# citibeth/spsparse

Hardware: NVIDIA B200
Metric: spgemm_intermediate_products_per_sec (higher is better)
Workload: dtype f64

## Files before the change

### spsparse_b200/csrc/radix_sort.cuh

```cuda
#pragma once
#include "common.cuh"

constexpr int RS_THREADS = 256;
#ifndef RS_IPT_N
#define RS_IPT_N 16
#endif
#ifndef RS_MIN_BLOCKS
#define RS_MIN_BLOCKS 3
#endif
constexpr int RS_IPT = RS_IPT_N;
constexpr int RS_HB = RS_IPT / 2;
constexpr int RS_TILE = RS_THREADS * RS_IPT;
constexpr int RS_WARPS = RS_THREADS / 32;
constexpr int RS_RADIX_BITS = 8;
constexpr int RS_RADIX = 1 << RS_RADIX_BITS;
constexpr int RS_NB = RS_RADIX + 1;
constexpr int RS_MAX_PASSES = 8;
#ifndef RS_LOOKBACK
#define RS_LOOKBACK 8
#endif
constexpr size_t RS_SMEM_BYTES =
    (size_t)RS_TILE * 16 + (size_t)RS_WARPS * RS_NB * sizeof(u32) + 64;

#define RS_WORD_AGG(c) ((c) + 1u)
// ... 218 lines not shown
                          input_kept(in, (u32)i, v[k]);
                key[h + k] = pack_key(hi[k], lo[k], in.bits_lo);
                valid_bits |= (ok ? 1u : 0u) << (h + k);
            }
        }
    } else if (BULK) {
        mbar_wait(&s_mbar[0], 0);
#pragma unroll
        for (int k = 0; k < RS_IPT; ++k) {
            const bool ok = wbase + (u64)k * 32 < n;
            key[k] = ok ? s_keys[warp * (32 * RS_IPT) + k * 32 + lane] : 0;
            valid_bits |= (ok ? 1u : 0u) << k;
        }
    } else {
#pragma unroll
        for (int k = 0; k < RS_IPT; ++k) {
            u64 i = wbase + (u64)k * 32;
            bool ok = i < n;
            key[k] = ok ? ld_stream_u64(a.keys_in + i) : 0;
            valid_bits |= (ok ? 1u : 0u) << k;
        }
#pragma unroll
        for (int k = 0; k < RS_IPT; ++k) {
            u64 i = wbase + (u64)k * 32;
            if (i < n && (lane & 15) == 0) asm volatile("prefetch.global.L2 [%0];" ::"l"(a.vals_in + i));
        }
    }

    u32 *mycnt = s_wcnt + warp * RS_NB;
    const u32 lt = lanemask_lt();
    unsigned short pos[RS_IPT];
#pragma unroll
    for (int k = 0; k < RS_IPT; ++k) {
        const bool ok = (valid_bits >> k) & 1u;
        const u32 d = (u32)((key[k] >> a.shift) & (RS_RADIX - 1));
        u32 peers;
        if (a.rank_mode == 0) {
            peers = __ballot_sync(SPB_FULL_MASK, ok);
#pragma unroll
            for (int b = 0; b < RS_RADIX_BITS; ++b) {
                int sgn;
                asm("bfe.s32 %0, %1, %2, 1;" : "=r"(sgn) : "r"(d), "r"(b));
                const u32 m = __ballot_sync(SPB_FULL_MASK, sgn != 0);
                peers &= ~(m ^ (u32)sgn);
            }
        } else {
            peers = __match_any_sync(SPB_FULL_MASK, ok ? d : (u32)RS_RADIX);
        }
        u32 leader = ok ? (u32)(__ffs(peers) - 1) : lane;
        u32 before = 0;
        if (ok && lane == leader) {
            before = mycnt[d];
            mycnt[d] = before + __popc(peers);
        }
        before = __shfl_sync(SPB_FULL_MASK, before, leader);
        pos[k] = (unsigned short)(before + __popc(peers & lt));
        __syncwarp();
    }
    __syncthreads();

    u32 total = 0;
#pragma unroll
    for (int w = 0; w < RS_WARPS; ++w) total += s_wcnt[w * RS_NB + tid];
    u32 *lb = a.lookback + (u64)tile * RS_RADIX + tid;
    st_relaxed_u32(lb, tile == 0 ? RS_WORD_INCL(total) : RS_WORD_AGG(total));
    u32 incl = warp_incl_scan(total);
    if (lane == 31) s_misc[1 + warp] = incl;
    __syncthreads();
    u32 lstart = incl - total;
    for (u32 w = 0; w < warp; ++w) lstart += s_misc[1 + w];
    const u32 nvalid_if_last = lstart + total;
    {
        u32 run = lstart;
#pragma unroll
        for (int w = 0; w < RS_WARPS; ++w) {
            u32 c = s_wcnt[w * RS_NB + tid];
            s_wcnt[w * RS_NB + tid] = run;
            run += c;
        }
    }
    if (tid == RS_RADIX - 1) s_misc[12] = nvalid_if_last;
    __syncthreads();
    const u32 nvalid = s_misc[12];

#pragma unroll
    for (int k = 0; k < RS_IPT; ++k) {
        if ((valid_bits >> k) & 1u) {
            u32 d = (u32)((key[k] >> a.shift) & (RS_RADIX - 1));
            u32 p = mycnt[d] + pos[k];
            pos[k] = (unsigned short)p;
            s_keys[p] = key[k];
        }
    }
    {
        const double *vsrc = PASS0 ? in.val : a.vals_in;
        double v[RS_IPT];
        if (BULK) {
            mbar_wait(&s_mbar[1], 0);
#pragma unroll
            for (int k = 0; k < RS_IPT; ++k) v[k] = s_vals[warp * (32 * RS_IPT) + k * 32 + lane];
            __syncthreads();
        } else {
#pragma unroll
            for (int k = 0; k < RS_IPT; ++k) {
                u64 i = wbase + (u64)k * 32;
                v[k] = ((valid_bits >> k) & 1u) ? ld_stream_f64(vsrc + i) : 0.0;
            }
        }
#pragma unroll
        for (int k = 0; k < RS_IPT; ++k)
            if ((valid_bits >> k) & 1u) s_vals[pos[k]] = v[k];
    }

    u32 excl = 0;
    if (tile > 0) {
        i64 p = (i64)tile - 1;
        bool done = false;
        while (!done) {
            u32 w[RS_LOOKBACK];
#pragma unroll
            for (int u = 0; u < RS_LOOKBACK; ++u)
                w[u] = (p - u >= 0) ? ld_relaxed_u32(a.lookback + (u64)(p - u) * RS_RADIX + tid) : RS_WORD_INCL(0u);
#pragma unroll
            for (int u = 0; u < RS_LOOKBACK; ++u) {
                if (done) break;
                while (!RS_READY(w[u])) w[u] = ld_relaxed_u32(a.lookback + (u64)(p - u) * RS_RADIX + tid);
                excl += RS_VALUE(w[u]);
                if (RS_IS_INCL(w[u])) done = true;
            }
            p -= RS_LOOKBACK;
        }
        st_relaxed_u32(lb, RS_WORD_INCL(excl + total));
    }
    const u32 gbase = a.bucket_start[tid] + excl - lstart;
    __syncthreads();
    s_wcnt[tid] = gbase;
    __syncthreads();

#pragma unroll
    for (int k = 0; k < RS_IPT; ++k) {
        u32 p = (u32)k * RS_THREADS + tid;
        if (p < nvalid) {
            u64 kk = s_keys[p];
            u32 dst = s_wcnt[(u32)((kk >> a.shift) & (RS_RADIX - 1))] + p;
            a.keys_out[dst] = kk;
            a.vals_out[dst] = s_vals[p];
        }
    }
}

constexpr int SG_THREADS = 256;
constexpr int SG_IPT = 8;
constexpr int SG_TILE = SG_THREADS * SG_IPT;
constexpr int SEG_MAX = 64;

constexpr int SG_CNT_SHIFT = 8;
__global__ void __launch_bounds__(SG_THREADS, 5) k_segment_sort(const u64 *__restrict__ keys_in, const double *__restrict__ vals_in,
                                                                const u32 *n_ptr, int bits_lo, u64 *keys_out, double *vals_out,
                                                                unsigned char *flags, u32 *long_count, u64 *tile_cnt = nullptr,
                                                                int keep_all = 0) {
    constexpr int W = SG_TILE + 2 * SEG_MAX;
    constexpr int ITS = (W + SG_THREADS - 1) / SG_THREADS;
    constexpr int NG = ITS * SG_THREADS / 32;
    __shared__ u64 s_key[W];
    __shared__ u32 s_col[W];
    __shared__ u32 s_hb[NG];
    __shared__ u32 s_last[NG];
    __shared__ u32 s_first[NG];
    const u32 n = *n_ptr;
    const u64 base = (u64)blockIdx.x * SG_TILE;
    if (base >= n) return;
    const u32 tid = threadIdx.x, lane = tid & 31, warp = tid >> 5;
    for (u32 q = tid; q < (u32)W; q += SG_THREADS) {
        const i64 g = (i64)base + (i64)q - SEG_MAX;
        s_key[q] = (g >= 0 && g < (i64)n) ? ld_stream_u64(keys_in + g) : ~0ull;
    }
#pragma unroll
    for (int k = 0; k < SG_IPT; ++k) {
        const u64 g = base + (u64)warp * 256 + (u64)k * 32 + lane;
        if (g < n && (lane & 15) == 0) asm volatile("prefetch.global.L2 [%0];" ::"l"(vals_in + g));
    }
    __syncthreads();
    const u64 lo_mask = (1ull << bits_lo) - 1;
#pragma unroll
    for (int it = 0; it < ITS; ++it) {
        const u32 q = (u32)it * SG_THREADS + tid;
        bool head = true;
        if (q < (u32)W) {
            const u64 kk = s_key[q];
            s_col[q] = (u32)(kk & lo_mask);
            head = q == 0 || (s_key[q - 1] >> bits_lo) != (kk >> bits_lo);
        }
        const u32 hb = __ballot_sync(SPB_FULL_MASK, head);
        if (lane == 0) {
            const u32 g = q >> 5;
            s_hb[g] = hb;
            s_last[g] = hb ? (g << 5) + 31 - __clz(hb) : 0;
            s_first[g] = hb ? (g << 5) + __ffs(hb) - 1 : 0xffffffffu;
        }
    }
    __syncthreads();
    if (warp == 0) {
        u32 carry = 0;
        for (int r = 0; r < (NG + 31) / 32; ++r) {
            const int g = r * 32 + (int)lane;
            const u32 mine = g < NG ? s_last[g] : 0;
            u32 inc = mine;
#pragma unroll
            for (int o = 1; o < 32; o <<= 1) {
                const u32 t = __shfl_up_sync(SPB_FULL_MASK, inc, o);
                if (lane >= (u32)o) inc = max(inc, t);
            }
            u32 exc = __shfl_up_sync(SPB_FULL_MASK, inc, 1);
            if (lane == 0) exc = 0;
            if (g < NG) s_last[g] = max(exc, carry);
            carry = max(carry, __shfl_sync(SPB_FULL_MASK, inc, 31));
        }
        carry = 0xffffffffu;
        for (int r = (NG + 31) / 32 - 1; r >= 0; --r) {
            const int g = r * 32 + (int)lane;
            const u32 mine = g < NG ? s_first[g] : 0xffffffffu;
            u32 inc = mine;
#pragma unroll
            for (int o = 1; o < 32; o <<= 1) {
                const u32 t = __shfl_down_sync(SPB_FULL_MASK, inc, o);
                if (lane + o < 32) inc = min(inc, t);
            }
            u32 exc = __shfl_down_sync(SPB_FULL_MASK, inc, 1);
            if (lane == 31) exc = 0xffffffffu;
            if (g < NG) s_first[g] = min(exc, carry);
            carry = min(carry, __shfl_sync(SPB_FULL_MASK, inc, 0));
        }
    }
    __syncthreads();
    u32 n_long = 0;
    i32 shift_by[SG_IPT];
    u32 cnt_at = 0, cnt_before = 0, cnt_after = 0;
    const u64 wbase = base + (u64)warp * 256;
#pragma unroll
    for (int k = 0; k < SG_IPT; ++k) {
        const u32 q = SEG_MAX + warp * 256 + (u32)k * 32 + lane;
        const u64 g = wbase + (u64)k * 32 + lane;
        shift_by[k] = 0;
        if (g < n) {
            bool head = true, rhead = false;
            const u32 grp = q >> 5, l = q & 31, hb = s_hb[grp];
            const u32 below = hb & (0xffffffffu >> (31 - l));
            const u32 st = below ? (grp << 5) + 31 - __clz(below) : s_last[grp];
            const u32 above = l < 31 ? hb & (0xffffffffu << (l + 1)) : 0u;
            const u32 nx = above ? (grp << 5) + __ffs(above) - 1 : s_first[grp];
            const bool is_long = nx - st > (u32)SEG_MAX;
            if (!is_long) {
                const u32 col = s_col[q];
                u32 before = 0, same = 0;
                for (u32 j = st; j < q; ++j) { before += s_col[j] <= col; same += s_col[j] == col; }
                for (u32 j = q + 1; j < nx; ++j) before += s_col[j] < col;
                shift_by[k] = (i32)(st + before) - (i32)q;
                head = keep_all || same == 0;
                rhead = before == 0;
            }
            if (flags) flags[g] = is_long;
            n_long += is_long;
            const u64 dst = (u64)((i64)g + shift_by[k]);
            const u32 inc = (head ? 1u : 0u) | (rhead ? 0x10000u : 0u);
            if (dst < wbase) cnt_before += inc;
            else if (dst >= wbase + 256) cnt_after += inc;
            else cnt_at += inc;
        }
    }
    if (tile_cnt) {
        const u32 a0 = __reduce_add_sync(SPB_FULL_MASK, cnt_at), a1 = __reduce_add_sync(SPB_FULL_MASK, cnt_before),
                  a2 = __reduce_add_sync(SPB_FULL_MASK, cnt_after);
        if (lane == 0) {
            u64 *t = tile_cnt + (wbase >> SG_CNT_SHIFT);
            if (a0) atomicAdd((ull *)t, (ull)(a0 & 0xffffu) | ((ull)(a0 >> 16) << 31));
            if (a1) atomicAdd((ull *)(t - 1), (ull)(a1 & 0xffffu) | ((ull)(a1 >> 16) << 31));
            if (a2) atomicAdd((ull *)(t + 1), (ull)(a2 & 0xffffu) | ((ull)(a2 >> 16) << 31));
        }
    }
    double v[SG_IPT];
#pragma unroll
    for (int k = 0; k < SG_IPT; ++k) {
        const u64 g = wbase + (u64)k * 32 + lane;
        v[k] = g < n ? ld_stream_f64(vals_in + g) : 0.0;
    }
#pragma unroll
    for (int k = 0; k < SG_IPT; ++k) {
        const u64 g = wbase + (u64)k * 32 + lane;
        if (g < n) {
            const u64 dst = (u64)((i64)g + shift_by[k]);
            keys_out[dst] = s_key[SEG_MAX + warp * 256 + k * 32 + lane];
            vals_out[dst] = v[k];
        }
    }
    n_long = __reduce_add_sync(SPB_FULL_MASK, n_long);
    if (n_long && lane == 0) atomicAdd(long_count, n_long);
}

static_assert(SG_TILE % 256 == 0 && (1 << SG_CNT_SHIFT) == 256, "a warp's 256 consecutive entries are one tile of the reduce pass");
#ifndef SGW_UNROLL_N
#define SGW_UNROLL_N 8
#endif
constexpr int SGW_UNROLL = SGW_UNROLL_N;
__global__ void __launch_bounds__(SG_THREADS, 6) k_segment_sort_walk(const u64 *__restrict__ keys_in, const double *__restrict__ vals_in,
                                                             const u32 *n_ptr, int bits_lo, u64 *keys_out, double *vals_out,
                                                             unsigned char *flags, u32 *long_count, u64 *tile_cnt = nullptr,
                                                             int keep_all = 0) {
    __shared__ u32 s_row[SG_TILE + 2 * SEG_MAX];
    __shared__ u32 s_col[SG_TILE + 2 * SEG_MAX];
    const u32 n = *n_ptr;
    const u64 base = (u64)blockIdx.x * SG_TILE;
    if (base >= n) return;
    const u32 tid = threadIdx.x;
    const u32 lo_mask = bits_lo >= 32 ? 0xffffffffu : (1u << bits_lo) - 1u;
    for (u32 q = tid; q < SG_TILE + 2 * SEG_MAX; q += SG_THREADS) {
        const i64 g = (i64)base + (i64)q - SEG_MAX;
        u32 row = 0xffffffffu, col = 0;
        if (g >= 0 && g < (i64)n) {
            const u64 key = ld_stream_u64(keys_in + g);
            row = (u32)(key >> bits_lo);
            col = (u32)key & lo_mask;
        }
        s_row[q] = row;
        s_col[q] = col;
    }
    const u32 lane = tid & 31, warp = tid >> 5;
    const u64 wbase = base + (u64)warp * 256;
    double v[SG_IPT];
#pragma unroll
    for (int k = 0; k < SG_IPT; ++k) {
        const u64 g = wbase + (u64)k * 32 + lane;
        v[k] = g < n ? ld_stream_f64(vals_in + g) : 0.0;
    }
    __syncthreads();
    u32 n_long = 0;
    u32 cnt_at = 0, cnt_before = 0, cnt_after = 0;
#pragma unroll
    for (int k = 0; k < SG_IPT; ++k) {
        const u32 q = SEG_MAX + warp * 256 + (u32)k * 32 + lane;
        const u64 g = wbase + (u64)k * 32 + lane;
        u64 dst = g;
        bool head = true, rhead = false;
        if (g < n) {
            const u32 row = s_row[q], col = s_col[q];
            u32 b = 0, f = 0, before = 0, same = 0;
            if (s_row[q - SEG_MAX] == row || s_row[q + SEG_MAX] == row) b = f = (u32)SEG_MAX;
            else {
#pragma unroll SGW_UNROLL
                for (b = 0; b < (u32)SEG_MAX; ++b) {
                    if (s_row[q - 1 - b] != row) break;
                    const u32 c = s_col[q - 1 - b];
                    before += c <= col;
                    same += c == col;
                }
#pragma unroll SGW_UNROLL
                for (f = 0; f < (u32)SEG_MAX; ++f) {
                    if (s_row[q + 1 + f] != row) break;
                    before += s_col[q + 1 + f] < col;
                }
            }
            const bool is_long = b == (u32)SEG_MAX || f == (u32)SEG_MAX || b + f + 1 > (u32)SEG_MAX;
            if (!is_long) {
                dst = g - b + before;
                head = keep_all || same == 0;
                rhead = before == 0;
            }
            keys_out[dst] = ((u64)row << bits_lo) | col;
            vals_out[dst] = v[k];
            if (flags) flags[g] = is_long;
            n_long += is_long;
            const u32 inc = (head ? 1u : 0u) | (rhead ? 0x10000u : 0u);
            if (dst < wbase) cnt_before += inc;
            else if (dst >= wbase + 256) cnt_after += inc;
            else cnt_at += inc;
        }
    }
    if (tile_cnt) {
        const u32 a0 = __reduce_add_sync(SPB_FULL_MASK, cnt_at), a1 = __reduce_add_sync(SPB_FULL_MASK, cnt_before),
                  a2 = __reduce_add_sync(SPB_FULL_MASK, cnt_after);
        if (lane == 0) {
            u64 *t = tile_cnt + (wbase >> SG_CNT_SHIFT);
            if (a0) atomicAdd((ull *)t, (ull)(a0 & 0xffffu) | ((ull)(a0 >> 16) << 31));
            if (a1) atomicAdd((ull *)(t - 1), (ull)(a1 & 0xffffu) | ((ull)(a1 >> 16) << 31));
            if (a2) atomicAdd((ull *)(t + 1), (ull)(a2 & 0xffffu) | ((ull)(a2 >> 16) << 31));
        }
    }
    n_long = __reduce_add_sync(SPB_FULL_MASK, n_long);
    if (n_long && lane == 0) atomicAdd(long_count, n_long);
}

constexpr int SGS_ROW = 5;
constexpr int SGS_H = SGS_ROW - 1;
constexpr int SGS_STEP = 32 - 2 * SGS_H;
constexpr int SGS_STEPS = (256 + SGS_STEP - 1) / SGS_STEP;
__global__ void __launch_bounds__(SG_THREADS, 6) k_segment_sort_shfl(const u64 *__restrict__ keys_in, const double *__restrict__ vals_in,
                                                                    const u32 *n_ptr, int bits_lo, u64 *keys_out, double *vals_out,
                                                                    unsigned char *flags, u32 *long_count, u64 *tile_cnt = nullptr,
                                                                    int keep_all = 0) {
    __shared__ u32 s_row[SG_TILE + 2 * SEG_MAX];
    __shared__ u32 s_col[SG_TILE + 2 * SEG_MAX];
    __shared__ double s_val[SG_TILE];
    const u32 n = *n_ptr;
    const u64 base = (u64)blockIdx.x * SG_TILE;
    if (base >= n) return;
    const u32 tid = threadIdx.x, lane = tid & 31, warp = tid >> 5;
    const u32 lo_mask = bits_lo >= 32 ? 0xffffffffu : (1u << bits_lo) - 1u;
    for (u32 q = tid; q < SG_TILE + 2 * SEG_MAX; q += SG_THREADS) {
        const i64 g = (i64)base + (i64)q - SEG_MAX;
        u32 row = 0xffffffffu, col = 0;
        if (g >= 0 && g < (i64)n) {
            const u64 key = ld_stream_u64(keys_in + g);
            row = (u32)(key >> bits_lo);
            col = (u32)key & lo_mask;
        }
        s_row[q] = row;
        s_col[q] = col;
    }
#pragma unroll
    for (int k = 0; k < SG_IPT; ++k) {
        const u32 e = (u32)k * SG_THREADS + tid;
        const u64 g = base + e;
        s_val[e] = g < n ? ld_stream_f64(vals_in + g) : 0.0;
    }
    __syncthreads();
    const u64 wbase = base + (u64)warp * 256;
    u32 n_long = 0;
    u32 cnt_at = 0, cnt_before = 0, cnt_after = 0;
    for (int t = 0; t < SGS_STEPS; ++t) {
        const i32 e = t * SGS_STEP + (i32)lane - SGS_H;
        const u32 q = (u32)(SEG_MAX + (i32)warp * 256 + e);
        const u64 g = wbase + (u64)(i64)e;
        const bool mine = lane >= (u32)SGS_H && lane < (u32)(32 - SGS_H) && e < 256 && g < n;
        const u32 row = s_row[q], col = s_col[q];
        const u32 hb = __ballot_sync(SPB_FULL_MASK, s_row[q - 1] != row);
        const u32 tail = __shfl_sync(SPB_FULL_MASK, (u32)(s_row[q + 1] != row), 31);
        const u64 z = ~((u64)hb | ((u64)tail << 32)) & 0x1ffffffffull;
        u64 run = z;
#pragma unroll
        for (int d = 1; d < SGS_ROW; ++d) run &= z >> d;
        u32 b = 0, f = 0, before = 0, same = 0;
        if (run == 0) {
#pragma unroll
            for (int d = 1; d < SGS_ROW; ++d) {
                const u32 ru = __shfl_up_sync(SPB_FULL_MASK, row, d), cu = __shfl_up_sync(SPB_FULL_MASK, col, d);
                const u32 rd = __shfl_down_sync(SPB_FULL_MASK, row, d), cd = __shfl_down_sync(SPB_FULL_MASK, col, d);
                const bool up = lane >= (u32)d && ru == row, dn = lane + d < 32u && rd == row;
                b += up;
                before += (up && cu <= col) + (dn && cd < col);
                same += up && cu == col;
                f += dn;
            }
        } else if (mine) {
            if (s_row[q - SEG_MAX] == row || s_row[q + SEG_MAX] == row) b = f = (u32)SEG_MAX;
            else {
                for (b = 0; b < (u32)SEG_MAX; ++b) {
                    if (s_row[q - 1 - b] != row) break;
                    const u32 c = s_col[q - 1 - b];
                    before += c <= col;
                    same += c == col;
                }
                for (f = 0; f < (u32)SEG_MAX; ++f) {
                    if (s_row[q + 1 + f] != row) break;
                    before += s_col[q + 1 + f] < col;
                }
            }
        }
        if (mine) {
            const bool is_long = b == (u32)SEG_MAX || f == (u32)SEG_MAX || b + f + 1 > (u32)SEG_MAX;
            u64 dst = g;
            bool head = true, rhead = false;
            if (!is_long) {
                dst = g - b + before;
                head = keep_all || same == 0;
                rhead = before == 0;
            }
            keys_out[dst] = ((u64)row << bits_lo) | col;
            vals_out[dst] = s_val[warp * 256 + (u32)e];
            if (flags) flags[g] = is_long;
            n_long += is_long;
            const u32 inc = (head ? 1u : 0u) | (rhead ? 0x10000u : 0u);
            if (dst < wbase) cnt_before += inc;
            else if (dst >= wbase + 256) cnt_after += inc;
            else cnt_at += inc;
        }
    }
    if (tile_cnt) {
        const u32 a0 = __reduce_add_sync(SPB_FULL_MASK, cnt_at), a1 = __reduce_add_sync(SPB_FULL_MASK, cnt_before),
                  a2 = __reduce_add_sync(SPB_FULL_MASK, cnt_after);
        if (lane == 0) {
            u64 *t = tile_cnt + (wbase >> SG_CNT_SHIFT);
            if (a0) atomicAdd((ull *)t, (ull)(a0 & 0xffffu) | ((ull)(a0 >> 16) << 31));
            if (a1) atomicAdd((ull *)(t - 1), (ull)(a1 & 0xffffu) | ((ull)(a1 >> 16) << 31));
            if (a2) atomicAdd((ull *)(t + 1), (ull)(a2 & 0xffffu) | ((ull)(a2 >> 16) << 31));
        }
    }
    n_long = __reduce_add_sync(SPB_FULL_MASK, n_long);
    if (n_long && lane == 0) atomicAdd(long_count, n_long);
}

__global__ void k_gather_flagged(const u64 *__restrict__ keys, const double *__restrict__ vals, const unsigned char *__restrict__ flags,
                                 const u64 *__restrict__ slot, u32 n, u64 *k_out, double *v_out) {
    for (u64 e = (u64)blockIdx.x * blockDim.x + threadIdx.x; e < n; e += (u64)gridDim.x * blockDim.x)
        if (flags[e]) { k_out[slot[e]] = keys[e]; v_out[slot[e]] = vals[e]; }
}
__global__ void k_scatter_flagged(const u64 *__restrict__ k_sorted, const double *__restrict__ v_sorted,
                                  const unsigned char *__restrict__ flags, const u64 *__restrict__ slot, u32 n, u64 *keys, double *vals) {
    for (u64 e = (u64)blockIdx.x * blockDim.x + threadIdx.x; e < n; e += (u64)gridDim.x * blockDim.x)
        if (flags[e]) { keys[e] = k_sorted[slot[e]]; vals[e] = v_sorted[slot[e]]; }
}
```

### spsparse_b200/csrc/reduce_segsort.cuh

```cuda
#pragma once
#include "radix_sort.cuh"
#include "reduce_by_key.cuh"

constexpr int RF_H = SEG_MAX;
constexpr int RF_W = RK_TILE + 2 * RF_H;
constexpr int RF_ITS = (RF_W + RK_THREADS - 1) / RK_THREADS;
constexpr int RF_SORTED = RK_TILE + RF_H + 1;
constexpr int RF_SLOTS = RF_SORTED + (RF_SORTED >> 3) + 1;

struct RfSmem {
    u64 raw[RF_W];
    u64 keys[RF_SLOTS];
    double vals[RF_SLOTS];
    u64 warp[RK_WARPS];
    u64 excl;
    u32 tile;
};

__global__ void __launch_bounds__(RK_THREADS, 4) k_reduce_segsort(ReduceArgs a, u32 *seg_long) {
    extern __shared__ __align__(16) unsigned char rf_smem[];
    RfSmem &s = *reinterpret_cast<RfSmem *>(rf_smem);
    const u32 tid = threadIdx.x, lane = tid & 31, warp = tid >> 5;
    const bool want_rows = a.row_start != nullptr;
    if (tid == 0) s.tile = atomicAdd(a.ticket, 1u);
    __syncthreads();
    const u32 tile = s.tile;
    const u32 n = *a.n_ptr;
    const u64 base = (u64)tile * RK_TILE;
    if (base >= n) return;
    const u32 tile_n = (n - base < (u64)RK_TILE) ? (u32)(n - base) : (u32)RK_TILE;

    double v[RF_ITS];
#pragma unroll
    for (int k = 0; k < RF_ITS; ++k) {
        const u32 q = (u32)k * RK_THREADS + tid;
        const i64 g = (i64)base + (i64)q - RF_H;
        const bool in = q < (u32)RF_W && g >= 0 && g < (i64)n;
        if (q < (u32)RF_W) s.raw[q] = in ? ld_stream_u64(a.keys + g) : ~0ull;
        v[k] = in ? ld_stream_f64(a.vals + g) : 0.0;
    }
    __syncthreads();

    const u64 lo_mask = (1ull << a.bits_lo) - 1;
    u32 n_long = 0;
#pragma unroll
    for (int k = 0; k < RF_ITS; ++k) {
        const u32 q = (u32)k * RK_THREADS + tid;
        if (q >= (u32)RF_W) continue;
        const u64 key = s.raw[q];
        if (key == ~0ull) continue;
        const u64 row = key >> a.bits_lo, col = key & lo_mask;
        u32 b = 0, f = 0, before = 0;
        bool cut = false;
        for (; b < (u32)SEG_MAX; ++b) {
            if (q < 1 + b) { cut = true; break; }
            const u64 kk = s.raw[q - 1 - b];
            if ((kk >> a.bits_lo) != row) break;
            before += (kk & lo_mask) <= col;
        }
        for (; f < (u32)SEG_MAX; ++f) {
            if (q + 1 + f >= (u32)RF_W) { cut = true; break; }
            const u64 kk = s.raw[q + 1 + f];
            if ((kk >> a.bits_lo) != row) break;
            before += (kk & lo_mask) < col;
        }
        const bool is_long = b == (u32)SEG_MAX || f == (u32)SEG_MAX || b + f + 1 > (u32)SEG_MAX;
        if (q >= (u32)RF_H && q < (u32)(RF_H + RK_TILE)) n_long += is_long;
        const u32 place = (cut || is_long) ? q : q - b + before;
        if (place + 1 >= (u32)RF_H && place + 1 < (u32)(RF_H + RF_SORTED)) {
            const u32 L = place + 1 - (u32)RF_H;
            s.keys[rk_phys(L)] = key;
            s.vals[rk_phys(L)] = v[k];
        }
    }
    n_long = __reduce_add_sync(SPB_FULL_MASK, n_long);
    if (n_long && lane == 0) atomicAdd(seg_long, n_long);
    __syncthreads();

    const u32 first = tid * RK_IPT;
    const u32 mine = first < tile_n ? (tile_n - first < (u32)RK_IPT ? tile_n - first : (u32)RK_IPT) : 0;
    u64 key[RK_IPT];
    double acc[RK_IPT];
    u32 head_bits = 0, rhead_bits = 0;
    if (mine) {
        const u64 prev = s.keys[rk_phys(first)];
#pragma unroll
        for (int j = 0; j < RK_IPT; ++j) {
            key[j] = s.keys[rk_phys(first + j + 1)];
            acc[j] = s.vals[rk_phys(first + j + 1)];
        }
        int cur = -1;
#pragma unroll
        for (int j = 0; j < RK_IPT; ++j) {
            if ((u32)j < mine) {
                const u64 before = j ? key[j - 1] : prev;
                const bool head = (a.policy == POLICY_KEEP_ALL) || (base + first + j == 0) || (key[j] != before);
                if (head) {
                    head_bits |= 1u << j;
                    if (want_rows && ((base + first + j == 0) || (key[j] >> a.bits_lo) != (before >> a.bits_lo)))
                        rhead_bits |= 1u << j;
                    cur = j;
                } else if (cur >= 0) {
                    const double vj = acc[j];
#pragma unroll
                    for (int h = 0; h < RK_IPT; ++h)
                        if (h == cur) {
                            if (a.policy == POLICY_ADD) acc[h] = __dadd_rn(acc[h], vj);
                            else if (a.policy == POLICY_REPLACE) acc[h] = vj;
                        }
                }
            }
        }
        if (cur >= 0 && mine == (u32)RK_IPT && (a.policy == POLICY_ADD || a.policy == POLICY_REPLACE)) {
            const u64 k0 = key[RK_IPT - 1];
            double sum = 0.0;
#pragma unroll
            for (int h = 0; h < RK_IPT; ++h) if (h == cur) sum = acc[h];
            u64 q = base + first + RK_IPT;
            while (q < n) {
                const u32 L = (u32)(q - base) + 1;
                if (L >= (u32)RF_SORTED) break;
                if (s.keys[rk_phys(L)] != k0) break;
                const double vq = s.vals[rk_phys(L)];
                if (a.policy == POLICY_ADD) sum = __dadd_rn(sum, vq); else sum = vq;
                ++q;
            }
#pragma unroll
            for (int h = 0; h < RK_IPT; ++h) if (h == cur) acc[h] = sum;
        }
    }
    const u32 emit_bits = head_bits;
    const u64 my = (u64)__popc(emit_bits) | ((u64)__popc(rhead_bits) << 32);
    const u64 incl = warp_incl_scan(my);
    if (lane == 31) s.warp[warp] = incl;
    __syncthreads();
    u64 wbefore = 0, total = 0;
#pragma unroll
    for (int w = 0; w < RK_WARPS; ++w) {
        const u64 t = s.warp[w];
        if ((u32)w < warp) wbefore += t;
        total += t;
    }
    const u64 before_me = wbefore + incl - my;
    const u32 tile_out = (u32)(total & 0xffffffffull);
    if (warp == 0) {
        const u64 packed = (total & 0xffffffffull) | ((total >> 32) << 31);
        const u64 excl0 = lookback_exclusive(a.state, tile, packed);
        if (lane == 0) {
            s.excl = excl0;
            if (base + RK_TILE >= n) {
                const u64 fin = excl0 + packed;
                const u32 n_out = (u32)(fin & 0x7fffffffull), n_rows = (u32)(fin >> 31);
                *a.out_count = n_out;
                if (want_rows) { *a.row_count = n_rows; a.row_start[n_rows] = n_out; }
            }
        }
    }
    {
        u32 slot = (u32)(before_me & 0xffffffffull);
#pragma unroll
        for (int j = 0; j < RK_IPT; ++j) {
            if ((emit_bits >> j) & 1u) {
                s.keys[slot] = key[j];
                s.vals[slot] = acc[j];
                ++slot;
            }
        }
    }
    __syncthreads();
    const u64 excl_rows = s.excl >> 31;
    const u64 excl = s.excl & 0x7fffffffull;
    if (rhead_bits) {
        u32 slot = (u32)(before_me & 0xffffffffull);
        u64 rslot = excl_rows + (before_me >> 32);
#pragma unroll
        for (int j = 0; j < RK_IPT; ++j) {
            if ((emit_bits >> j) & 1u) {
                if ((rhead_bits >> j) & 1u) {
                    a.row_start[rslot] = (u32)(excl + slot);
                    a.row_id[rslot] = (i32)(key[j] >> a.bits_lo);
                    ++rslot;
                }
                ++slot;
            }
        }
    }
    for (u32 t = tid; t < tile_out; t += RK_THREADS) {
        const u64 k = s.keys[t];
        a.out_hi[excl + t] = (i32)(k >> a.bits_lo);
        if (a.out_lo) a.out_lo[excl + t] = (i32)(k & lo_mask);
        a.out_val[excl + t] = s.vals[t];
    }
}
```

### spsparse_b200/csrc/spb_api.cu

```cuda
#include "../../include/spsparse_b200.h"

#include <cstdarg>
#include <cstdio>
#include <cstdlib>
#include <cstring>
#include <chrono>
#include <map>
#include <mutex>
#include <thread>
#include <unordered_map>
#include <vector>

#include "common.cuh"
#include "csr.cuh"
#include "gen.cuh"
#include "radix_sort.cuh"
#include "radix_sort9.cuh"
#include "reduce_by_key.cuh"
#include "reduce_segsort.cuh"
#include "reduce_warp.cuh"
#include "scan.cuh"
#include "spgemm.cuh"
#include "dense_ops.cuh"
#include "rowpart.cuh"

thread_local std::string g_last_error;

int spb_fail(int code, const char *fmt, ...) {
    char buf[1024];
    va_list ap;
    va_start(ap, fmt);
    vsnprintf(buf, sizeof buf, fmt, ap);
    va_end(ap);
    g_last_error = buf;
    return code;
}

static inline double now_ms() {
    return std::chrono::duration<double, std::milli>(std::chrono::steady_clock::now().time_since_epoch()).count();
}
static double g_alloc_ms = 0;
static int g_trace = -1;
static inline bool tracing() {
    if (g_trace < 0) g_trace = getenv("SPB_TRACE") ? 1 : 0;
    return g_trace == 1;
}

struct DevPool {
    std::multimap<size_t, void *> free_;
    std::unordered_map<void *, size_t> live_;
    std::mutex mu_;
    size_t cached_bytes = 0;

    static size_t round_up(size_t b) {
        if (b < 512) return 512;
        if (b < (1u << 20)) return (b + 511) & ~(size_t)511;
        return (b + (1u << 20) - 1) & ~(size_t)((1u << 20) - 1);
    }
    cudaError_t alloc(void **out, size_t bytes) {
        std::lock_guard<std::mutex> g(mu_);
        const size_t want = round_up(bytes);
        auto it = free_.lower_bound(want);
        if (it != free_.end() && it->first <= want + (want >= (64u << 20) ? want / 2 : want / 8)) {
            *out = it->second;
            live_[*out] = it->first;
            cached_bytes -= it->first;
            free_.erase(it);
            return cudaSuccess;
        }
        void *p = nullptr;
        cudaError_t e = cudaMalloc(&p, want);
        if (e != cudaSuccess) {
            cudaGetLastError();
            trim_locked();
            e = cudaMalloc(&p, want);
            if (e != cudaSuccess) return e;
        }
        live_[p] = want;
        *out = p;
        return cudaSuccess;
    }
    void release(void *p) {
        if (!p) return;
        std::lock_guard<std::mutex> g(mu_);
        auto it = live_.find(p);
        if (it == live_.end()) return;
        free_.insert({it->second, p});
        cached_bytes += it->second;
        live_.erase(it);
    }
    void trim_locked() {
        cudaDeviceSynchronize();
        for (auto &kv : free_) cudaFree(kv.second);
        free_.clear();
        cached_bytes = 0;
    }
    void destroy() {
        std::lock_guard<std::mutex> g(mu_);
        trim_locked();
        for (auto &kv : live_) cudaFree(kv.first);
        live_.clear();
    }
};

struct spb_ctx {
    int device;
    cudaStream_t stream;
    bool own_stream;
    int sm_count;
    u32 merge_max_products;
    u64 esc_chunk;
    u64 hash_min_products;
    int hash_variant;
    u64 launches;
    bool bulk_load;
    static constexpr int XFER_WORKERS = 8;
    int xfer_workers;
    static constexpr size_t XFER_CHUNK = 16u << 20;
    void *xfer_buf[XFER_WORKERS][2];
    cudaStream_t xfer_stream[XFER_WORKERS];
    cudaEvent_t xfer_ev[XFER_WORKERS][2];
    bool xfer_ready;
    DevPool pool;
};

struct spb_coo {
    int rank;
    u64 shape[2];
    u64 n;
    i32 *idx[2];
    double *val;
    int sort_order[2];
    bool owned;
    u32 *row_start;
    i32 *row_id;
    u32 nrows;
    bool rows_valid;
    u32 *dense_ptr;
    bool dense_ptr_owned;
    u32 *range_ptr;
    u64 range_lo, range_hi;
    u32 max_row_len;
};

struct Scratch {
    spb_ctx *ctx;
    std::vector<void *> ptrs;
    explicit Scratch(spb_ctx *c) : ctx(c) {}
    ~Scratch() { for (void *p : ptrs) ctx->pool.release(p); }
    template <typename T>
    int get(T **out, u64 count) {
        void *p = nullptr;
        size_t bytes = (size_t)(count ? count : 1) * sizeof(T);
        double t0 = tracing() ? now_ms() : 0;
        cudaError_t e = ctx->pool.alloc(&p, bytes);
        if (tracing()) { double dt = now_ms() - t0; g_alloc_ms += dt; if (dt > 1.0) fprintf(stderr, "[spb] pool.alloc(%zu MB) took %.2f ms\n", bytes >> 20, dt); }
        if (e != cudaSuccess) return spb_fail(SPB_ERR_CUDA, "device allocation of %zu bytes failed: %s", bytes, cudaGetErrorString(e));
        ptrs.push_back(p);
        *out = (T *)p;
        return 0;
    }
    template <typename T>
    int zeroed(T **out, u64 count) {
        CKR(get(out, count));
        CK(cudaMemsetAsync(*out, 0, (size_t)(count ? count : 1) * sizeof(T), ctx->stream));
        return 0;
    }
    void release(void *p) {
        for (size_t i = 0; i < ptrs.size(); ++i)
            if (ptrs[i] == p) { ctx->pool.release(p); ptrs.erase(ptrs.begin() + i); return; }
    }
    void keep(void *p) {
        for (size_t i = 0; i < ptrs.size(); ++i)
            if (ptrs[i] == p) { ptrs.erase(ptrs.begin() + i); return; }
    }
};

struct Timer {
    cudaStream_t s;
    std::vector<cudaEvent_t> ev;
    explicit Timer(cudaStream_t st) : s(st) {}
    ~Timer() { for (auto e : ev) cudaEventDestroy(e); }
    int mark() {
        cudaEvent_t e;
        cudaEventCreate(&e);
        cudaEventRecord(e, s);
        ev.push_back(e);
        return (int)ev.size() - 1;
    }
    float ms(int a, int b) {
        float t = 0;
        cudaEventSynchronize(ev[b]);
        cudaEventElapsedTime(&t, ev[a], ev[b]);
        return t;
    }
};

static inline u32 grid_for(u64 n, u32 threads, u32 cap) {
    u64 g = div_up(n ? n : 1, threads);
    return (u32)(g < cap ? g : cap);
}

static bool host_ptr_is_pinned(const void *p) {
    cudaPointerAttributes at;
    if (cudaPointerGetAttributes(&at, p) != cudaSuccess) { cudaGetLastError(); return false; }
    return at.type == cudaMemoryTypeHost || at.type == cudaMemoryTypeManaged;
}

static int xfer_setup(spb_ctx *c) {
    if (c->xfer_ready) return 0;
    {
        int want = getenv("SPB_XFER_WORKERS") ? atoi(getenv("SPB_XFER_WORKERS")) : (int)(std::thread::hardware_concurrency() / 2);
        c->xfer_workers = want < 1 ? 1 : (want > spb_ctx::XFER_WORKERS ? spb_ctx::XFER_WORKERS : want);
    }
    for (int w = 0; w < c->xfer_workers; ++w) {
        CK(cudaStreamCreateWithFlags(&c->xfer_stream[w], cudaStreamNonBlocking));
        for (int b = 0; b < 2; ++b) {
            CK(cudaHostAlloc(&c->xfer_buf[w][b], spb_ctx::XFER_CHUNK, cudaHostAllocDefault));
            CK(cudaEventCreateWithFlags(&c->xfer_ev[w][b], cudaEventDisableTiming));
        }
    }
    c->xfer_ready = true;
    return 0;
}

struct XferJob { void *dev; void *host; size_t bytes; };

static int staged_copy(spb_ctx *c, const XferJob *jobs, int njobs, bool to_device) {
    bool all_pinned = true;
    size_t total = 0;
    for (int j = 0; j < njobs; ++j) { if (jobs[j].bytes) { all_pinned = all_pinned && host_ptr_is_pinned(jobs[j].host); total += jobs[j].bytes; } }
    if (all_pinned || total < (4u << 20)) {
        for (int j = 0; j < njobs; ++j)
            if (jobs[j].bytes)
                CK(cudaMemcpyAsync(to_device ? jobs[j].dev : jobs[j].host, to_device ? jobs[j].host : jobs[j].dev, jobs[j].bytes,
                                   to_device ? cudaMemcpyHostToDevice : cudaMemcpyDeviceToHost, c->stream));
        CK(cudaStreamSynchronize(c->stream));
        return 0;
    }
    CKR(xfer_setup(c));
    struct Chunk { char *dev; char *host; size_t bytes; };
    std::vector<Chunk> chunks;
    for (int j = 0; j < njobs; ++j)
        for (size_t o = 0; o < jobs[j].bytes; o += spb_ctx::XFER_CHUNK)
            chunks.push_back({(char *)jobs[j].dev + o, (char *)jobs[j].host + o, std::min(spb_ctx::XFER_CHUNK, jobs[j].bytes - o)});
    const int NW = c->xfer_workers;
    cudaError_t err[spb_ctx::XFER_WORKERS];
    auto work = [&](int w) {
        cudaError_t e = cudaSetDevice(c->device);
        int b = 0;
        size_t pending_chunk[2] = {(size_t)-1, (size_t)-1};
        for (size_t k = w; k < chunks.size() && e == cudaSuccess; k += (size_t)NW, b ^= 1) {
            const Chunk &ch = chunks[k];
            if (to_device) {
                e = cudaEventSynchronize(c->xfer_ev[w][b]);
                if (e != cudaSuccess) break;
                memcpy(c->xfer_buf[w][b], ch.host, ch.bytes);
                e = cudaMemcpyAsync(ch.dev, c->xfer_buf[w][b], ch.bytes, cudaMemcpyHostToDevice, c->xfer_stream[w]);
                if (e == cudaSuccess) e = cudaEventRecord(c->xfer_ev[w][b], c->xfer_stream[w]);
            } else {
                e = cudaMemcpyAsync(c->xfer_buf[w][b], ch.dev, ch.bytes, cudaMemcpyDeviceToHost, c->xfer_stream[w]);
                if (e == cudaSuccess) e = cudaEventRecord(c->xfer_ev[w][b], c->xfer_stream[w]);
                pending_chunk[b] = k;
                const int o = b ^ 1;
                if (e == cudaSuccess && pending_chunk[o] != (size_t)-1) {
                    e = cudaEventSynchronize(c->xfer_ev[w][o]);
                    if (e == cudaSuccess) memcpy(chunks[pending_chunk[o]].host, c->xfer_buf[w][o], chunks[pending_chunk[o]].bytes);
                    pending_chunk[o] = (size_t)-1;
                }
            }
        }
        if (!to_device)
            for (int o = 0; o < 2 && e == cudaSuccess; ++o)
                if (pending_chunk[o] != (size_t)-1) {
                    e = cudaEventSynchronize(c->xfer_ev[w][o]);
                    if (e == cudaSuccess) memcpy(chunks[pending_chunk[o]].host, c->xfer_buf[w][o], chunks[pending_chunk[o]].bytes);
                }
        if (e == cudaSuccess) e = cudaStreamSynchronize(c->xfer_stream[w]);
        err[w] = e;
    };
    CK(cudaStreamSynchronize(c->stream));
    std::thread th[spb_ctx::XFER_WORKERS];
    for (int w = 1; w < NW; ++w) th[w] = std::thread(work, w);
    work(0);
    for (int w = 1; w < NW; ++w) th[w].join();
    for (int w = 0; w < NW; ++w)
        if (err[w] != cudaSuccess) return spb_fail(SPB_ERR_CUDA, "host transfer failed: %s", cudaGetErrorString(err[w]));
    return 0;
}

extern "C" {

const char *spb_last_error(void) { return g_last_error.c_str(); }
int spb_version(void) { return 100; }

int spb_ctx_create(int device, void *cuda_stream, spb_ctx **out) {
    if (!out) return spb_fail(SPB_ERR_ARG, "spb_ctx_create: out is null");
    int count = 0;
    cudaError_t e = cudaGetDeviceCount(&count);
    if (e != cudaSuccess || count == 0)
        return spb_fail(SPB_ERR_CUDA, "no CUDA device available (%s); spsparse_b200 has no CPU fallback",
                        cudaGetErrorString(e));
    if (device < 0 || device >= count) return spb_fail(SPB_ERR_ARG, "device %d out of range (%d devices)", device, count);
    CK(cudaSetDevice(device));
    struct Undo {
        spb_ctx *c;
        ~Undo() {
            if (!c) return;
            if (c->own_stream && c->stream) cudaStreamDestroy(c->stream);
            delete c;
        }
    } undo{new spb_ctx()};
    spb_ctx *c = undo.c;
    c->device = device;
    c->stream = nullptr;
    c->own_stream = (cuda_stream == nullptr);
    if (c->own_stream) CK(cudaStreamCreateWithFlags(&c->stream, cudaStreamNonBlocking));
    else c->stream = (cudaStream_t)cuda_stream;
    CK(cudaDeviceGetAttribute(&c->sm_count, cudaDevAttrMultiProcessorCount, device));
    CK(cudaFuncSetAttribute(k_radix_pass<true>, cudaFuncAttributeMaxDynamicSharedMemorySize, (int)RS_SMEM_BYTES));
    CK(cudaFuncSetAttribute(k_radix_pass<false>, cudaFuncAttributeMaxDynamicSharedMemorySize, (int)RS_SMEM_BYTES));
    CK(cudaFuncSetAttribute(k_reduce_segsort, cudaFuncAttributeMaxDynamicSharedMemorySize, (int)sizeof(RfSmem)));
    CK(cudaFuncSetAttribute(k_radix_pass9<true>, cudaFuncAttributeMaxDynamicSharedMemorySize, (int)R9_SMEM_BYTES));
    CK(cudaFuncSetAttribute(k_radix_pass9<false>, cudaFuncAttributeMaxDynamicSharedMemorySize, (int)R9_SMEM_BYTES));
    CK(cudaFuncSetAttribute(k_radix_pass<false, true>, cudaFuncAttributeMaxDynamicSharedMemorySize, (int)RS_SMEM_BYTES));
    CK(cudaFuncSetAttribute(k_radix_pass<true, true>, cudaFuncAttributeMaxDynamicSharedMemorySize, (int)RS_SMEM_BYTES));
    CK(cudaFuncSetAttribute(k_radix_pass9<true, true>, cudaFuncAttributeMaxDynamicSharedMemorySize, (int)R9_SMEM_BYTES));
    CK(cudaFuncSetAttribute(k_radix_pass9<false, true>, cudaFuncAttributeMaxDynamicSharedMemorySize, (int)R9_SMEM_BYTES));
    c->bulk_load = getenv("SPB_BULK_LOAD") ? atoi(getenv("SPB_BULK_LOAD")) != 0 : true;
    const char *s = getenv("SPB_MERGE_MAX_PRODUCTS");
    c->merge_max_products = s ? (u32)strtoul(s, nullptr, 10) : 1024u;
    s = getenv("SPB_ESC_CHUNK");
    c->esc_chunk = s ? strtoull(s, nullptr, 10) : (1ull << 27);
    c->launches = 0;
    c->xfer_ready = false;
    s = getenv("SPB_HASH_MIN_PRODUCTS");
    c->hash_min_products = s ? (strcmp(s, "off") == 0 ? ~0ull : strtoull(s, nullptr, 10)) : 512ull;
    s = getenv("SPB_HASH_VARIANT");
    c->hash_variant = s ? atoi(s) : 2;
    CK(cudaFuncSetAttribute(k_hash_symbolic, cudaFuncAttributeMaxDynamicSharedMemorySize, (int)(HASH_MAX_COLS / 8)));
    CK(cudaFuncSetAttribute(k_hash_numeric<1024, 10240, 16384>, cudaFuncAttributeMaxDynamicSharedMemorySize, (int)sizeof(HashSmem<1024, 10240, 16384>)));
    CK(cudaFuncSetAttribute(k_hash_numeric<512, 5120, 8192>, cudaFuncAttributeMaxDynamicSharedMemorySize, (int)sizeof(HashSmem<512, 5120, 8192>)));
    CK(cudaFuncSetAttribute(k_hash_numeric<256, 2560, 4096>, cudaFuncAttributeMaxDynamicSharedMemorySize, (int)sizeof(HashSmem<256, 2560, 4096>)));
    if (c->esc_chunk < 1) c->esc_chunk = 1;
    undo.c = nullptr;
    *out = c;
    return SPB_OK;
}

int spb_ctx_destroy(spb_ctx *ctx) {
    if (!ctx) return SPB_OK;
    cudaSetDevice(ctx->device);
    cudaStreamSynchronize(ctx->stream);
    if (ctx->xfer_ready)
        for (int w = 0; w < ctx->xfer_workers; ++w) {
            cudaStreamDestroy(ctx->xfer_stream[w]);
            for (int b = 0; b < 2; ++b) { cudaFreeHost(ctx->xfer_buf[w][b]); cudaEventDestroy(ctx->xfer_ev[w][b]); }
        }
    ctx->pool.destroy();
    if (ctx->own_stream) cudaStreamDestroy(ctx->stream);
    delete ctx;
    return SPB_OK;
}

int spb_ctx_sync(spb_ctx *ctx) {
    if (!ctx) return spb_fail(SPB_ERR_ARG, "null context");
    CK(cudaStreamSynchronize(ctx->stream));
    return SPB_OK;
}

int spb_ctx_trim(spb_ctx *ctx, uint64_t *released_bytes) {
    if (!ctx) return spb_fail(SPB_ERR_ARG, "null context");
    CK(cudaSetDevice(ctx->device));
    std::lock_guard<std::mutex> g(ctx->pool.mu_);
    if (released_bytes) *released_bytes = ctx->pool.cached_bytes;
    ctx->pool.trim_locked();
    return SPB_OK;
}

int spb_host_prefault(void *p, uint64_t bytes) {
    if (!p || !bytes) return SPB_OK;
    unsigned nt = std::thread::hardware_concurrency();
    if (nt > 16) nt = 16;
    if (bytes < (64ull << 20) || nt < 2) nt = 1;
    constexpr uint64_t PAGE = 4096;
    auto work = [=](unsigned t) {
        volatile char *c = static_cast<volatile char *>(p);
        const uint64_t a = bytes * t / nt, b = bytes * (t + 1) / nt;
        if (a < b) c[a] = 0;
        const uint64_t base = reinterpret_cast<uintptr_t>(p);
        for (uint64_t o = ((base + a + PAGE - 1) & ~(PAGE - 1)) - base; o < b; o += PAGE) c[o] = 0;
    };
    if (nt == 1) { work(0); return SPB_OK; }
    std::vector<std::thread> th;
    for (unsigned t = 1; t < nt; ++t) th.emplace_back(work, t);
    work(0);
    for (auto &x : th) x.join();
    return SPB_OK;
}

int spb_ctx_launch_count(const spb_ctx *ctx, uint64_t *launches) {
    if (!ctx || !launches) return spb_fail(SPB_ERR_ARG, "null argument");
    *launches = ctx->launches;
    return SPB_OK;
}

int spb_ctx_device(const spb_ctx *ctx, int *device, void **cuda_stream) {
    if (!ctx) return spb_fail(SPB_ERR_ARG, "null context");
    if (device) *device = ctx->device;
    if (cuda_stream) *cuda_stream = (void *)ctx->stream;
    return SPB_OK;
}

static int coo_new(spb_ctx *ctx, int rank, const u64 *shape, u64 n, bool allocate, spb_coo **out) {
    if (!ctx || !out || !shape) return spb_fail(SPB_ERR_ARG, "null argument");
    if (rank != 1 && rank != 2) return spb_fail(SPB_ERR_ARG, "rank must be 1 or 2 (got %d)", rank);
    for (int k = 0; k < rank; ++k)
        if (shape[k] > (1ull << 31)) return spb_fail(SPB_ERR_ARG, "extent %llu exceeds the int32 index range", (ull)shape[k]);
    if (n >= (1ull << 31)) return spb_fail(SPB_ERR_TOO_LARGE, "%llu entries: the reference's own cap is 2^31 (algorithm.hpp:419)", (ull)n);
    spb_coo *a = new spb_coo();
    a->rank = rank;
    a->shape[0] = shape[0];
    a->shape[1] = rank > 1 ? shape[1] : 1;
    a->n = n;
    a->idx[0] = a->idx[1] = nullptr;
    a->val = nullptr;
    a->sort_order[0] = -1;
    a->sort_order[1] = 0;
    a->owned = allocate;
    a->row_start = nullptr;
    a->row_id = nullptr;
    a->nrows = 0;
    a->rows_valid = false;
    a->dense_ptr = nullptr;
    a->dense_ptr_owned = true;
    a->range_ptr = nullptr;
    a->range_lo = a->range_hi = 0;
    a->max_row_len = 0;
    if (allocate) {
        size_t cnt = n ? n : 1;
        cudaError_t e = cudaSetDevice(ctx->device);
        for (int k = 0; k < rank && e == cudaSuccess; ++k) e = ctx->pool.alloc((void **)&a->idx[k], cnt * sizeof(i32));
        if (e == cudaSuccess) e = ctx->pool.alloc((void **)&a->val, cnt * sizeof(double));
        if (e != cudaSuccess) {
            for (int k = 0; k < 2; ++k) ctx->pool.release(a->idx[k]);
            ctx->pool.release(a->val);
            delete a;
            return spb_fail(SPB_ERR_CUDA, "device allocation for %llu entries failed: %s", (ull)n, cudaGetErrorString(e));
        }
    }
    *out = a;
    return SPB_OK;
}

static void drop_row_cache(spb_ctx *ctx, spb_coo *a) {
    if (ctx) {
        ctx->pool.release(a->row_start);
        ctx->pool.release(a->row_id);
        if (a->dense_ptr_owned) ctx->pool.release(a->dense_ptr);
        ctx->pool.release(a->range_ptr);
    }
    a->row_start = nullptr; a->row_id = nullptr; a->dense_ptr = nullptr; a->range_ptr = nullptr;
    a->rows_valid = false; a->nrows = 0; a->max_row_len = 0;
}

static void set_order(spb_coo *a, const int *so) {
    a->sort_order[0] = -1;
    a->sort_order[1] = 0;
    if (so && so[0] >= 0) {
        a->sort_order[0] = so[0];
        a->sort_order[1] = a->rank > 1 ? so[1] : 0;
    }
}

int spb_coo_alloc(spb_ctx *ctx, int rank, const uint64_t *shape, uint64_t n, spb_coo **out) {
    return coo_new(ctx, rank, shape, n, true, out);
}

int spb_coo_upload(spb_ctx *ctx, int rank, const uint64_t *shape, const int32_t *const *idx, const double *val,
                   uint64_t n, const int *sort_order, spb_coo **out) {
    if (n && (!idx || !val)) return spb_fail(SPB_ERR_ARG, "null data pointer");
    CKR(coo_new(ctx, rank, shape, n, true, out));
    spb_coo *a = *out;
    set_order(a, sort_order);
    XferJob jobs[3];
    int nj = 0;
    for (int k = 0; k < rank && n; ++k) {
        if (!idx[k]) { spb_coo_free(ctx, a); *out = nullptr; return spb_fail(SPB_ERR_ARG, "null index pointer for dimension %d", k); }
        jobs[nj++] = {a->idx[k], const_cast<int32_t *>(idx[k]), (size_t)n * sizeof(i32)};
    }
    if (n) jobs[nj++] = {a->val, const_cast<double *>(val), (size_t)n * sizeof(double)};
    const int rc = nj ? staged_copy(ctx, jobs, nj, true) : 0;
    if (rc) {
        spb_coo_free(ctx, a);
        *out = nullptr;
        return rc;
    }
    return SPB_OK;
}

int spb_coo_wrap_device(spb_ctx *ctx, int rank, const uint64_t *shape, int32_t *const *d_idx, double *d_val,
                        uint64_t n, const int *sort_order, spb_coo **out) {
    if (n && (!d_idx || !d_val)) return spb_fail(SPB_ERR_ARG, "null device pointer");
    CKR(coo_new(ctx, rank, shape, n, false, out));
    spb_coo *a = *out;
    for (int k = 0; k < rank; ++k) a->idx[k] = d_idx ? d_idx[k] : nullptr;
    a->val = d_val;
    set_order(a, sort_order);
    return SPB_OK;
}

int spb_coo_info(const spb_coo *a, int *rank, uint64_t *shape, uint64_t *n, int *sort_order) {
    if (!a) return spb_fail(SPB_ERR_ARG, "null array");
    if (rank) *rank = a->rank;
    for (int k = 0; k < a->rank; ++k) {
        if (shape) shape[k] = a->shape[k];
        if (sort_order) sort_order[k] = a->sort_order[k];
    }
    if (n) *n = a->n;
    return SPB_OK;
}

int spb_coo_device_ptrs(const spb_coo *a, int32_t **d_idx, double **d_val) {
    if (!a) return spb_fail(SPB_ERR_ARG, "null array");
    for (int k = 0; k < a->rank; ++k) if (d_idx) d_idx[k] = a->idx[k];
    if (d_val) *d_val = a->val;
    return SPB_OK;
}

int spb_coo_set_sorted(spb_coo *a, const int *sort_order) {
    if (!a) return spb_fail(SPB_ERR_ARG, "null array");
    if (a->rows_valid || a->dense_ptr)
        return spb_fail(SPB_ERR_ARG, "spb_coo_set_sorted: the array's row structure is already in use");
    set_order(a, sort_order);
    return SPB_OK;
}

int spb_coo_download(spb_ctx *ctx, const spb_coo *a, int32_t *const *idx, double *val) {
    if (!ctx || !a) return spb_fail(SPB_ERR_ARG, "null argument");
    CK(cudaSetDevice(ctx->device));
    XferJob jobs[3];
    int nj = 0;
    if (a->n) {
        for (int k = 0; k < a->rank; ++k)
            if (idx && idx[k]) jobs[nj++] = {a->idx[k], idx[k], (size_t)a->n * sizeof(i32)};
        if (val) jobs[nj++] = {a->val, val, (size_t)a->n * sizeof(double)};
    }
    if (nj) return staged_copy(ctx, jobs, nj, false);
    CK(cudaStreamSynchronize(ctx->stream));
    return SPB_OK;
}

int spb_coo_free(spb_ctx *ctx, spb_coo *a) {
    if (!a) return SPB_OK;
    if (a->owned && ctx) {
        for (int k = 0; k < 2; ++k) if (a->idx[k]) ctx->pool.release(a->idx[k]);
        if (a->val) ctx->pool.release(a->val);
    }
    drop_row_cache(ctx, a);
    delete a;
    return SPB_OK;
}

}

struct SortJob {
    SortInput in;
    int bits_hi;
    int policy;
};

template <typename InT, typename OutT>
static int exclusive_scan(spb_ctx *ctx, Scratch &ws, const InT *in, OutT *out, u64 n);

static int run_radix_passes(spb_ctx *ctx, Scratch &ws, int first_pass, int passes, u32 n_cap, const u32 *n_ptr,
                            u32 *hist, u64 *kA, double *vA, u64 *kB, double *vB, const SortInput *in0,
                            u64 **keys_sorted, double **vals_sorted, Timer *tm, int *mark_after_first, int shift0 = 0,
                            int digit_bits = RS_RADIX_BITS) {
    const u32 tiles = (u32)div_up(n_cap ? n_cap : 1, RS_TILE);
    const bool nine = digit_bits == R9_BITS;
    const u64 radix = nine ? R9_RADIX : RS_RADIX;
    u32 *lookback, *tickets;
    CKR(ws.zeroed(&lookback, (u64)passes * tiles * radix));
    CKR(ws.zeroed(&tickets, (u64)passes));
    u64 *kin = kA, *kout = kB;
    double *vin = vA, *vout = vB;
    for (int p = 0; p < passes; ++p) {
        PassArgs a;
        a.n_ptr = n_ptr;
        a.bucket_start = hist + (u64)p * radix;
        a.lookback = lookback + (u64)p * tiles * radix;
        a.ticket = tickets + p;
        a.shift = shift0 + p * digit_bits;
        a.rank_mode = getenv("SPB_RANK_MODE") ? atoi(getenv("SPB_RANK_MODE")) : 0;
        if (p == 0 && first_pass == 0) {
            a.keys_in = nullptr; a.vals_in = nullptr; a.keys_out = kA; a.vals_out = vA;
            const bool aligned = ((((uintptr_t)in0->hi) | ((uintptr_t)in0->lo) | ((uintptr_t)in0->val)) & 15u) == 0;
            const u32 tiles_bulk = (ctx->bulk_load && aligned) ? n_cap / RS_TILE : 0;
            if (tiles_bulk) {
                ++ctx->launches;
                if (nine) k_radix_pass9<true, true><<<tiles_bulk, RS_THREADS, R9_SMEM_BYTES, ctx->stream>>>(a, *in0);
                else k_radix_pass<true, true><<<tiles_bulk, RS_THREADS, RS_SMEM_BYTES, ctx->stream>>>(a, *in0);
            }
            if (tiles > tiles_bulk) {
                ++ctx->launches;
                if (nine) k_radix_pass9<true><<<tiles - tiles_bulk, RS_THREADS, R9_SMEM_BYTES, ctx->stream>>>(a, *in0);
                else k_radix_pass<true><<<tiles - tiles_bulk, RS_THREADS, RS_SMEM_BYTES, ctx->stream>>>(a, *in0);
            }
            kin = kA; vin = vA; kout = kB; vout = vB;
            if (tm) *mark_after_first = tm->mark();
        } else {
            a.keys_in = kin; a.vals_in = vin; a.keys_out = kout; a.vals_out = vout;
            SortInput dummy;
            memset(&dummy, 0, sizeof dummy);
            ++ctx->launches;
            if (ctx->bulk_load) {
                if (nine) k_radix_pass9<false, true><<<tiles, RS_THREADS, R9_SMEM_BYTES, ctx->stream>>>(a, dummy);
                else k_radix_pass<false, true><<<tiles, RS_THREADS, RS_SMEM_BYTES, ctx->stream>>>(a, dummy);
            } else {
                if (nine) k_radix_pass9<false><<<tiles, RS_THREADS, R9_SMEM_BYTES, ctx->stream>>>(a, dummy);
                else k_radix_pass<false><<<tiles, RS_THREADS, RS_SMEM_BYTES, ctx->stream>>>(a, dummy);
            }
            u64 *tk = kin; kin = kout; kout = tk;
            double *tv = vin; vin = vout; vout = tv;
        }
    }
    CK(cudaGetLastError());
    *keys_sorted = kin;
    *vals_sorted = vin;
    return 0;
}

static int sort_reduce(spb_ctx *ctx, const SortJob &job, i32 *out_hi, i32 *out_lo, double *out_val,
                       u32 *h_kept, u32 *h_out, spb_consolidate_stats *st, u32 *row_start = nullptr,
                       i32 *row_id = nullptr, u32 *h_rows = nullptr) {
    const SortInput &in = job.in;
    const u32 n = in.n;
    const int key_bits = job.bits_hi + in.bits_lo;
    int passes_full = (key_bits + RS_RADIX_BITS - 1) / RS_RADIX_BITS;
    if (passes_full < 1) passes_full = 1;
    if (passes_full > RS_MAX_PASSES) return spb_fail(SPB_ERR_ARG, "key of %d bits is too wide", key_bits);
    int passes_row = (job.bits_hi + RS_RADIX_BITS - 1) / RS_RADIX_BITS;
    if (passes_row < 1) passes_row = 1;
    const char *seg_env = getenv("SPB_SEGMENT_SORT");
    const bool seg_short = (double)n <= 16.0 * (double)in.extent_hi && n >= (1u << 23);
    const char *walk_env = getenv("SPB_SEGMENT_WALK");
    const bool seg_walk = walk_env ? atoi(walk_env) != 0 : (double)n <= 6.0 * (double)in.extent_hi;
    const bool seg_shfl = walk_env && atoi(walk_env) == 2;
    const bool seg = in.bits_lo > 0 && passes_full - passes_row >= 2 &&
                     (seg_env ? atoi(seg_env) != 0 : seg_short);
    const int cover_bits = seg ? job.bits_hi : key_bits;
    const char *r9_env = getenv("SPB_RADIX9");
    const int passes8 = seg ? passes_row : passes_full;
    const int passes9 = cover_bits > 0 ? (cover_bits + R9_BITS - 1) / R9_BITS : 1;
    const bool nine_wanted = r9_env ? atoi(r9_env) != 0 : (seg && !seg_env);
    const bool nine = nine_wanted && passes9 < passes8;
    const int digit_bits = nine ? R9_BITS : RS_RADIX_BITS;
    const int passes = nine ? passes9 : passes8;
    const int shift0 = seg ? in.bits_lo : 0;
    if (n >= (1u << 31)) return spb_fail(SPB_ERR_TOO_LARGE, "%u entries: one sort holds fewer than 2^31 (the reference's own cap, algorithm.hpp:419)", n);
    Scratch ws(ctx);
    Timer tm(ctx->stream);
    const int t0 = tm.mark();

    u32 *hist, *counters;
    u64 *first_kept;
    CKR(ws.zeroed(&hist, (u64)passes * (nine ? R9_RADIX : RS_RADIX)));
    CKR(ws.zeroed(&counters, 8));
    CKR(ws.get(&first_kept, 2));
    CK(cudaMemsetAsync(first_kept, 0xFF, 2 * sizeof(u64), ctx->stream));
    SortInput in0 = in;
    in0.first_kept = first_kept;
    const u32 sgrid = (u32)ctx->sm_count * 4;
    if (in.drop_nan) {
        ++ctx->launches, k_first_kept_key<<<grid_for(n, 256, sgrid * 2), 256, 0, ctx->stream>>>(in0, first_kept);
        ++ctx->launches, k_first_kept_pos<<<grid_for(n, 256, sgrid * 2), 256, 0, ctx->stream>>>(in0, first_kept);
    }
    const bool vec4 = ((((uintptr_t)in0.hi) | ((uintptr_t)in0.lo) | ((uintptr_t)in0.val)) & 15u) == 0 && n >= 4096 &&
                      !(getenv("SPB_VEC_LOAD") && atoi(getenv("SPB_VEC_LOAD")) == 0);
    if (nine) {
        ++ctx->launches;
        if (vec4) k_sort_hist_v4<9><<<grid_for(n / 4, 512, sgrid), 512, 0, ctx->stream>>>(in0, passes, shift0, hist, counters);
        else k_sort_hist9<<<grid_for(n, 512, sgrid), 512, 0, ctx->stream>>>(in0, passes, shift0, hist, counters);
        ++ctx->launches, k_bucket_starts9<<<passes, R9_RADIX / 2, 0, ctx->stream>>>(hist);
    } else {
        ++ctx->launches;
        if (vec4) k_sort_hist_v4<8><<<grid_for(n / 4, 512, sgrid), 512, 0, ctx->stream>>>(in0, passes, shift0, hist, counters);
        else k_sort_hist<<<grid_for(n, 512, sgrid), 512, 0, ctx->stream>>>(in0, passes, shift0, hist, counters);
        ++ctx->launches, k_bucket_starts<<<passes, RS_RADIX, 0, ctx->stream>>>(hist);
    }
    CK(cudaGetLastError());

    u64 *kA, *kB = nullptr, *ks;
    double *vA, *vB = nullptr, *vs;
    CKR(ws.get(&kA, n));
    CKR(ws.get(&vA, n));
    if (passes > 1 || seg) { CKR(ws.get(&kB, n)); CKR(ws.get(&vB, n)); }
    int t_p0 = t0;
    CKR(run_radix_passes(ctx, ws, 0, passes, n, counters, hist, kA, vA, kB, vB, &in0, &ks, &vs, &tm, &t_p0, shift0, digit_bits));
    const int t_passes = tm.mark();
    const char *fused_env = getenv("SPB_FUSED_REDUCE");
    bool fused = seg && seg_walk && fused_env && atoi(fused_env) != 0;
    u32 h[6];
    int t1 = t_passes, t2 = t_passes;
    u64 *const ks_rows = ks;
    double *const vs_rows = vs;
    bool long_rows_fixed = false;
    const int rw_mode = getenv("SPB_REDUCE_WARP") ? atoi(getenv("SPB_REDUCE_WARP")) : 1;
    const u32 wtiles = (u32)div_up(div_up(n ? n : 1, RW_TILE), RW_WARPS) * RW_WARPS;
    for (int attempt = 0;; ++attempt) {
        ks = ks_rows; vs = vs_rows;
        u64 *ko = (ks == kA) ? kB : kA;
        double *vo = (vs == vA) ? vB : vA;
        const u32 stiles = (u32)div_up(n, SG_TILE);
        u64 *tile_off = nullptr;
        if (seg && !fused) {
            if (!long_rows_fixed) {
                u64 *tile_cnt = nullptr;
                if (rw_mode == 1) {
                    CKR(ws.zeroed(&tile_cnt, (u64)wtiles + 2));
                    CKR(ws.get(&tile_off, (u64)wtiles + 2));
                }
                const int keep_all = job.policy == POLICY_KEEP_ALL;
                ++ctx->launches;
                if (seg_shfl) k_segment_sort_shfl<<<stiles, SG_THREADS, 0, ctx->stream>>>(ks, vs, counters, in.bits_lo, ko, vo, nullptr, counters + 5, tile_cnt, keep_all);
                else if (seg_walk) k_segment_sort_walk<<<stiles, SG_THREADS, 0, ctx->stream>>>(ks, vs, counters, in.bits_lo, ko, vo, nullptr, counters + 5, tile_cnt, keep_all);
                else k_segment_sort<<<stiles, SG_THREADS, 0, ctx->stream>>>(ks, vs, counters, in.bits_lo, ko, vo, nullptr, counters + 5, tile_cnt, keep_all);
                CK(cudaGetLastError());
                if (tile_cnt) CKR((exclusive_scan<u64, u64>(ctx, ws, tile_cnt, tile_off, (u64)wtiles + 1)));
            } else {
                const u32 n_kept = h[0], h_long = h[5];
                unsigned char *flags;
                u64 *slot, *lk, *lk2, *lks;
                double *lv, *lv2, *lvs;
                u32 *lhist, *lcount;
                CKR(ws.get(&flags, n_kept));
                CKR(ws.get(&slot, (u64)n_kept + 1));
                CK(cudaMemsetAsync(counters + 5, 0, sizeof(u32), ctx->stream));
                ++ctx->launches;
                if (seg_shfl) k_segment_sort_shfl<<<stiles, SG_THREADS, 0, ctx->stream>>>(ks, vs, counters, in.bits_lo, ko, vo, flags, counters + 5);
                else if (seg_walk) k_segment_sort_walk<<<stiles, SG_THREADS, 0, ctx->stream>>>(ks, vs, counters, in.bits_lo, ko, vo, flags, counters + 5);
                else k_segment_sort<<<stiles, SG_THREADS, 0, ctx->stream>>>(ks, vs, counters, in.bits_lo, ko, vo, flags, counters + 5);
                CKR((exclusive_scan<unsigned char, u64>(ctx, ws, flags, slot, n_kept)));
                CKR(ws.get(&lk, h_long)); CKR(ws.get(&lv, h_long)); CKR(ws.get(&lk2, h_long)); CKR(ws.get(&lv2, h_long));
                CKR(ws.zeroed(&lhist, (u64)passes_full * RS_RADIX));
                CKR(ws.zeroed(&lcount, 8));
                CK(cudaMemcpyAsync(lcount, &h_long, sizeof(u32), cudaMemcpyHostToDevice, ctx->stream));
                ++ctx->launches, k_gather_flagged<<<grid_for(n_kept, 256, sgrid * 4), 256, 0, ctx->stream>>>(ks, vs, flags, slot, n_kept, lk, lv);
                ++ctx->launches, k_keys_hist<<<grid_for(h_long, 512, sgrid), 512, 0, ctx->stream>>>(lk, h_long, passes_full, lhist);
                ++ctx->launches, k_bucket_starts<<<passes_full, RS_RADIX, 0, ctx->stream>>>(lhist);
                CKR(run_radix_passes(ctx, ws, 1, passes_full, h_long, lcount, lhist, lk, lv, lk2, lv2, nullptr, &lks, &lvs, nullptr, nullptr));
                ++ctx->launches, k_scatter_flagged<<<grid_for(n_kept, 256, sgrid * 4), 256, 0, ctx->stream>>>(lks, lvs, flags, slot, n_kept, ko, vo);
                CK(cudaGetLastError());
            }
            ks = ko; vs = vo;
        }
        t1 = tm.mark();

        const bool rwarp = !fused && (tile_off != nullptr || rw_mode == 2);
        const u32 rtiles = rwarp ? wtiles / RW_WARPS : (u32)div_up(n, RK_TILE);
        ReduceArgs ra;
        memset(&ra, 0, sizeof ra);
        ra.keys = ks; ra.vals = vs; ra.n_ptr = counters; ra.bits_lo = in.bits_lo; ra.policy = job.policy;
        ra.out_hi = out_hi; ra.out_lo = out_lo; ra.out_val = out_val; ra.out_count = counters + 2;
        if (tile_off) ra.state = tile_off;
        else CKR(ws.zeroed(&ra.state, rwarp ? (u64)wtiles : (u64)rtiles));
        CKR(ws.zeroed(&ra.ticket, 1));
        ra.long_cap = n / RK_LONG_RUN + 1;
        CKR(ws.get(&ra.long_list, 2ull * ra.long_cap));
        ra.long_count = counters + 3;
        ra.row_start = row_start; ra.row_id = row_id; ra.row_count = counters + 4;
        if (fused) {
            ++ctx->launches, k_reduce_segsort<<<rtiles, RK_THREADS, sizeof(RfSmem), ctx->stream>>>(ra, counters + 5);
        } else {
            if (rwarp && tile_off) ++ctx->launches, k_reduce_warp<false><<<rtiles, RW_THREADS, 0, ctx->stream>>>(ra);
            else if (rwarp) ++ctx->launches, k_reduce_warp<true><<<rtiles, RW_THREADS, 0, ctx->stream>>>(ra);
            else ++ctx->launches, k_reduce_by_key<MODE_CONSOLIDATE><<<rtiles, RK_THREADS, 0, ctx->stream>>>(ra);
            if (job.policy == POLICY_ADD || job.policy == POLICY_REPLACE)
                ++ctx->launches, k_long_runs<<<(u32)ctx->sm_count * 4, 256, 0, ctx->stream>>>(ra);
        }
        CK(cudaGetLastError());
        t2 = tm.mark();

        CK(cudaMemcpyAsync(h, counters, sizeof h, cudaMemcpyDeviceToHost, ctx->stream));
        CK(cudaStreamSynchronize(ctx->stream));
        if (h[5] && !h[1] && attempt == 0 && seg) {
            fused = false;
            long_rows_fixed = true;
            CK(cudaMemsetAsync(counters + 2, 0, 3 * sizeof(u32), ctx->stream));
            continue;
        }
        break;
    }
    if (h[1]) return spb_fail(SPB_ERR_ARG, "Sparse index out of bounds (an index is negative or >= its extent)");
    *h_kept = h[0];
    *h_out = h[2];
    if (h_rows) *h_rows = h[4];
    if (st) {
        st->n_in = n; st->n_kept = h[0]; st->n_out = h[2];
        st->key_bits = key_bits; st->passes = passes; st->digit_bits = digit_bits;
        st->ms_sort = tm.ms(t0, t1); st->ms_reduce = tm.ms(t1, t2); st->ms_total = tm.ms(t0, t2);
        st->ms_pass = passes > 1 ? tm.ms(t_p0, t_passes) / (float)(passes - 1) : 0.f;
    }
    return 0;
}

static int consolidate_core(spb_ctx *ctx, const spb_coo *in, const int *so, const int *ref_so, int policy,
                            bool drop_zero, int zero_nan, spb_coo **out, spb_consolidate_stats *st,
                            i32 *ext_lo = nullptr, double *ext_val = nullptr) {
    if (in->n >= (1ull << 31)) return spb_fail(SPB_ERR_TOO_LARGE, "%llu entries: one array holds fewer than 2^31 (the reference's own cap, algorithm.hpp:419)", (ull)in->n);
    spb_coo *r = nullptr;
    if (ext_lo && ext_val && in->rank == 2) {
        CKR(coo_new(ctx, in->rank, in->shape, in->n, false, &r));
        r->owned = true;
        if (ctx->pool.alloc((void **)&r->idx[so[0]], (in->n ? in->n : 1) * sizeof(i32)) != cudaSuccess) {
            delete r;
            return spb_fail(SPB_ERR_CUDA, "out of device memory");
        }
        r->idx[so[1]] = ext_lo;
        r->val = ext_val;
    } else {
        CKR(coo_new(ctx, in->rank, in->shape, in->n, true, &r));
    }
    set_order(r, so);
    if (st) memset(st, 0, sizeof *st);
    if (in->n == 0) { *out = r; return SPB_OK; }
    const int d0 = so[0], d1 = in->rank > 1 ? so[1] : -1;
    SortJob job;
    memset(&job, 0, sizeof job);
    job.in.hi = in->idx[d0];
    job.in.lo = d1 >= 0 ? in->idx[d1] : nullptr;
    job.in.val = in->val;
    job.in.n = (u32)in->n;
    job.in.bits_lo = d1 >= 0 ? bits_for(in->shape[d1]) : 0;
    job.in.extent_hi = (u32)(in->shape[d0] > 0xffffffffull ? 0xffffffffu : in->shape[d0]);
    job.in.extent_lo = d1 >= 0 ? (u32)in->shape[d1] : 1u;
    job.in.drop_zero = drop_zero ? 1 : 0;
    job.in.drop_nan = (drop_zero && zero_nan) ? 1 : 0;
    const int r0 = ref_so[0], r1 = in->rank > 1 ? ref_so[1] : -1;
    job.in.ref_hi = in->idx[r0];
    job.in.ref_lo = r1 >= 0 ? in->idx[r1] : nullptr;
    job.in.ref_bits_lo = r1 >= 0 ? bits_for(in->shape[r1]) : 0;
    job.bits_hi = bits_for(in->shape[d0]);
    job.policy = policy;
    u32 kept = 0, nout = 0, nrows = 0;
    if (in->rank == 2) {
        const u64 cap = (in->n < in->shape[d0] ? in->n : in->shape[d0]) + 1;
        if (ctx->pool.alloc((void **)&r->row_start, cap * sizeof(u32)) != cudaSuccess ||
            ctx->pool.alloc((void **)&r->row_id, cap * sizeof(i32)) != cudaSuccess) {
            spb_coo_free(ctx, r);
            return spb_fail(SPB_ERR_CUDA, "out of device memory");
        }
    }
    int rc = sort_reduce(ctx, job, r->idx[d0], d1 >= 0 ? r->idx[d1] : nullptr, r->val, &kept, &nout, st,
                         r->row_start, r->row_id, &nrows);
    if (rc) { spb_coo_free(ctx, r); return rc; }
    r->n = nout;
    if (in->rank == 2) {
        r->nrows = nrows;
        r->rows_valid = true;
        if (nout == 0) { const u32 z = 0; cudaMemcpyAsync(r->row_start, &z, sizeof z, cudaMemcpyHostToDevice, ctx->stream); }
    }
    *out = r;
    return SPB_OK;
}

static int check_order(const spb_coo *a, const int *so, const char *what) {
    if (!so) return spb_fail(SPB_ERR_ARG, "%s: sort_order is null", what);
    for (int k = 0; k < a->rank; ++k)
        if (a->n && !a->idx[k]) return spb_fail(SPB_ERR_ARG, "%s: array is in compressed (pointer) form", what);
    bool seen[2] = {false, false};
    for (int k = 0; k < a->rank; ++k) {
        if (so[k] < 0 || so[k] >= a->rank || seen[so[k]])
            return spb_fail(SPB_ERR_ARG, "%s: sort_order is not a permutation of the dimensions", what);
        seen[so[k]] = true;
    }
    return 0;
}

struct RowIndex {
    u32 *start;
    i32 *id;
    u32 nrows;
};

static int build_row_index(spb_ctx *ctx, const spb_coo *a_const, RowIndex *ri) {
    spb_coo *a = const_cast<spb_coo *>(a_const);
    if (!a->rows_valid && a->n && !a->idx[a->sort_order[0]])
        return spb_fail(SPB_ERR_ARG, "array in compressed (pointer) form has no row list; use it as the B operand only");
    if (!a->rows_valid) {
        const u32 n = (u32)a->n;
        const i32 *hi = a->idx[a->sort_order[0]];
        Scratch ws(ctx);
        u32 *rs = nullptr;
        i32 *rid = nullptr;
        CK(ctx->pool.alloc((void **)&rs, ((u64)n + 1) * sizeof(u32)));
        if (ctx->pool.alloc((void **)&rid, ((u64)n + 1) * sizeof(i32)) != cudaSuccess) {
            ctx->pool.release(rs);
            return spb_fail(SPB_ERR_CUDA, "out of device memory (row list of %u entries)", n);
        }
        a->row_start = rs; a->row_id = rid;
        u32 *count, *ticket;
        u64 *state;
        const u32 tiles = (u32)div_up(n ? n : 1, RH_TILE);
        CKR(ws.zeroed(&count, 1));
        CKR(ws.zeroed(&ticket, 1));
        CKR(ws.zeroed(&state, tiles));
        if (n) ++ctx->launches, k_row_heads<<<tiles, RH_THREADS, 0, ctx->stream>>>(hi, n, a->row_start, a->row_id, count, state, ticket);
        ++ctx->launches, k_row_sentinel<<<1, 1, 0, ctx->stream>>>(a->row_start, count, n);
        CK(cudaGetLastError());
        CK(cudaMemcpyAsync(&a->nrows, count, sizeof(u32), cudaMemcpyDeviceToHost, ctx->stream));
        CK(cudaStreamSynchronize(ctx->stream));
        a->rows_valid = true;
    }
    ri->start = a->row_start;
    ri->id = a->row_id;
    ri->nrows = a->nrows;
    return 0;
}

template <typename InT, typename OutT>
static int exclusive_scan(spb_ctx *ctx, Scratch &ws, const InT *in, OutT *out, u64 n) {
    if (n == 0) { CK(cudaMemsetAsync(out, 0, sizeof(OutT), ctx->stream)); return 0; }
    const u32 tiles = (u32)div_up(n, SC_TILE);
    u64 *state;
    u32 *ticket;
    CKR(ws.zeroed(&state, tiles));
    CKR(ws.zeroed(&ticket, 1));
    ++ctx->launches, k_exclusive_scan<InT, OutT><<<tiles, SC_THREADS, 0, ctx->stream>>>(in, out, n, state, ticket);
    CK(cudaGetLastError());
    return 0;
}

static int build_dense_ptr(spb_ctx *ctx, const spb_coo *a_const, u64 extent, u32 **ptr_out) {
    spb_coo *a = const_cast<spb_coo *>(a_const);
    if (!a->dense_ptr) {
        RowIndex ri;
        CKR(build_row_index(ctx, a, &ri));
        CK(ctx->pool.alloc((void **)&a->dense_ptr, (extent + 2) * sizeof(u32)));
        Scratch ws(ctx);
        DpGap *gaps = nullptr;
        u32 *n_gaps = nullptr;
        if (ri.nrows && extent + 1 - ri.nrows >= DP_LONG_GAP) {
            CKR(ws.get(&gaps, (extent + 1) / DP_LONG_GAP + 1));
            CKR(ws.zeroed(&n_gaps, 1));
        }
        ++ctx->launches;
        if (ri.nrows) k_dense_ptr_from_rows<<<grid_for(ri.nrows, 256, (u32)ctx->sm_count * 16), 256, 0, ctx->stream>>>(ri.start, ri.id, ri.nrows, (u32)a->n, extent, a->dense_ptr, gaps, n_gaps);
        else k_fill_u32<<<grid_for(extent + 1, 256, (u32)ctx->sm_count * 16), 256, 0, ctx->stream>>>(a->dense_ptr, extent + 1, 0u);
        if (gaps) ++ctx->launches, k_fill_gaps<<<(u32)ctx->sm_count * 8, 256, 0, ctx->stream>>>(gaps, n_gaps, a->dense_ptr);
        CK(cudaGetLastError());
    }
    *ptr_out = a->dense_ptr;
    return 0;
}

static int densify(spb_ctx *ctx, Scratch &ws, const spb_coo *v, u64 dim, double **dense, unsigned char **mask, u32 *bad) {
    CKR(ws.zeroed(dense, dim));
    if (mask) CKR(ws.zeroed(mask, dim));
    if (v->n) ++ctx->launches, k_densify<<<grid_for(v->n, 256, 1u << 16), 256, 0, ctx->stream>>>(v->idx[0], v->val, v->n, dim, *dense, mask ? *mask : nullptr, bad);
    CK(cudaGetLastError());
    return 0;
}
static int bad_scale_vector() {
    return spb_fail(SPB_ERR_ARG, "a scale vector (or a vector operand flagged sorted) is not strictly ascending in its index: the "
                    "reference joins these as sorted lists without repeats (xiter.hpp:146, 201)");
}

static int esc_sort_reduce(spb_ctx *ctx, u64 *kA, double *vA, u32 count, int key_bits, int kbits,
                           const MMOperands &m, u32 row_lo, i32 *t_row, i32 *t_k, double *t_v, u32 *h_out) {
    Scratch ws(ctx);
    int passes = (key_bits + RS_RADIX_BITS - 1) / RS_RADIX_BITS;
    if (passes < 1) passes = 1;
    u32 *hist, *counters;
    CKR(ws.zeroed(&hist, (u64)passes * RS_RADIX));
    CKR(ws.zeroed(&counters, 8));
    CK(cudaMemcpyAsync(counters, &count, sizeof(u32), cudaMemcpyHostToDevice, ctx->stream));
    ++ctx->launches, k_keys_hist<<<grid_for(count, 512, (u32)ctx->sm_count * 4), 512, 0, ctx->stream>>>(kA, count, passes, hist);
    ++ctx->launches, k_bucket_starts<<<passes, RS_RADIX, 0, ctx->stream>>>(hist);
    u64 *kB, *ks;
    double *vB, *vs;
    CKR(ws.get(&kB, count));
    CKR(ws.get(&vB, count));
    {
        const u32 tiles = (u32)div_up(count, RS_TILE);
        u32 *lookback, *tickets;
        CKR(ws.zeroed(&lookback, (u64)passes * tiles * RS_RADIX));
        CKR(ws.zeroed(&tickets, (u64)passes));
        u64 *kin = kA, *kout = kB;
        double *vin = vA, *vout = vB;
        SortInput dummy;
        memset(&dummy, 0, sizeof dummy);
        for (int p = 0; p < passes; ++p) {
            PassArgs a;
            a.keys_in = kin; a.vals_in = vin; a.keys_out = kout; a.vals_out = vout;
            a.n_ptr = counters;
            a.bucket_start = hist + (u64)p * RS_RADIX;
            a.lookback = lookback + (u64)p * tiles * RS_RADIX;
            a.ticket = tickets + p;
            a.shift = p * RS_RADIX_BITS;
            a.rank_mode = 0;
        a.rank_mode = getenv("SPB_RANK_MODE") ? atoi(getenv("SPB_RANK_MODE")) : 0;
            ++ctx->launches;
            if (ctx->bulk_load) k_radix_pass<false, true><<<tiles, RS_THREADS, RS_SMEM_BYTES, ctx->stream>>>(a, dummy);
            else k_radix_pass<false><<<tiles, RS_THREADS, RS_SMEM_BYTES, ctx->stream>>>(a, dummy);
            u64 *tk = kin; kin = kout; kout = tk;
            double *tv = vin; vin = vout; vout = tv;
        }
        ks = kin; vs = vin;
        CK(cudaGetLastError());
    }
    const u32 rtiles = (u32)div_up(count, RK_TILE);
    ReduceArgs ra;
    memset(&ra, 0, sizeof ra);
    ra.keys = ks; ra.vals = vs; ra.n_ptr = counters; ra.bits_lo = kbits; ra.policy = POLICY_ADD;
    ra.out_hi = t_row; ra.out_lo = t_k; ra.out_val = t_v; ra.out_count = counters + 2;
    CKR(ws.zeroed(&ra.state, rtiles));
    CKR(ws.zeroed(&ra.ticket, 1));
    ra.row_ids = m.arow_id; ra.row_base = (i32)row_lo; ra.si = m.si; ra.sk = m.sk; ra.C = m.C;
    ++ctx->launches, k_reduce_by_key<MODE_ESC><<<rtiles, RK_THREADS, 0, ctx->stream>>>(ra);
    CK(cudaGetLastError());
    CK(cudaMemcpyAsync(h_out, counters + 2, sizeof(u32), cudaMemcpyDeviceToHost, ctx->stream));
    CK(cudaStreamSynchronize(ctx->stream));
    return 0;
}

struct EscChunk { i32 *row; i32 *k; double *v; u32 n; };

static size_t ballast_for_blocks(int blocks_per_sm, size_t static_smem) {
    if (blocks_per_sm <= 0) return 0;
    const size_t per = (size_t)(227 * 1024) / (size_t)blocks_per_sm;
    return per > static_smem + 1024 ? per - static_smem - 1024 : 0;
}
template <typename K> static int allow_ballast(K kernel) {
    static thread_local const void *done[16];
    static thread_local int n = 0;
    for (int i = 0; i < n; ++i) if (done[i] == (const void *)kernel) return 0;
    CK(cudaFuncSetAttribute(kernel, cudaFuncAttributeMaxDynamicSharedMemorySize, 200 * 1024));
    if (n < 16) done[n++] = (const void *)kernel;
    return 0;
}

struct PreScale {
    const double *sj;
    const unsigned char *sj_mask;
};

static int multiply_core(spb_ctx *ctx, double C, const spb_coo *si, const spb_coo *A, int a_row_dim,
                         const spb_coo *sj, const spb_coo *B, int b_inner_dim, const spb_coo *sk,
                         spb_coo *out, spb_mm_stats *st, Timer &tm, int t_begin, bool symbolic_only = false,
                         const PreScale *pre = nullptr) {
    Scratch ws(ctx);
    const int a_in = 1 - a_row_dim, b_col = 1 - b_inner_dim;
    const u64 m_rows = A->shape[a_row_dim], n_inner = A->shape[a_in], n_cols = B->shape[b_col];
    MMOperands m;
    memset(&m, 0, sizeof m);
    m.C = C;
    m.debug = getenv("SPB_MERGE_DEBUG") ? atoi(getenv("SPB_MERGE_DEBUG")) : 0;
    m.a_j = A->idx[a_in]; m.a_val = A->val; m.nnz_a = (u32)A->n;
    RowIndex ri;
    CKR(build_row_index(ctx, A, &ri));
    m.arow_id = ri.id; m.arow_start = ri.start; m.nrows = ri.nrows;
    u32 *bptr;
    CKR(build_dense_ptr(ctx, B, n_inner, &bptr));
    m.bptr = bptr; m.b_k = B->idx[b_col]; m.b_val = B->val;
    double *d;
    unsigned char *mask;
    u32 *bad_vec;
    CKR(ws.zeroed(&bad_vec, 1));
    if (si) { CKR(densify(ctx, ws, si, m_rows, &d, nullptr, bad_vec)); m.si = d; }
    if (pre) { m.sj = pre->sj; m.sj_mask = pre->sj_mask; }
    else if (sj) { CKR(densify(ctx, ws, sj, n_inner, &d, &mask, bad_vec)); m.sj = d; m.sj_mask = mask; }
    if (sk) { CKR(densify(ctx, ws, sk, n_cols, &d, nullptr, bad_vec)); m.sk = d; }
    const int t_prep = tm.mark();
    double h0 = now_ms();
    if (tracing()) fprintf(stderr, "[spb] mm: prepare done (host), alloc so far %.2f ms\n", g_alloc_ms);

    const u32 nrows = m.nrows;
    u32 *row_cnt;
    u64 *ent_off = nullptr, *esc_f = nullptr, *esc_off, *c_ptr;
    unsigned char *row_cls;
    ull *stats;
    CKR(ws.get(&row_cls, nrows));
    CKR(ws.zeroed(&row_cnt, (u64)nrows + 1));
    ull *mstats;
    CKR(ws.zeroed(&stats, 8));
    CKR(ws.zeroed(&mstats, (u64)MC_STRIPES * 8));
    const u32 cap = (u32)ctx->sm_count * 32;
    {
        const double avg_a_len = nrows ? (double)m.nnz_a / (double)nrows : 0.0;
// ... 1391 lines not shown
```

Baseline: 43.64 billion.

## Replace last radix pass with in-block group sort over low row bits

Adds a k_group_sort kernel that, when groups of consecutive row-bit buckets are expected to fit in a 4096-entry shared-memory tile, sorts each group in shared memory on up to 9 low row bits and then runs the per-row column walk. This lets the global radix sort skip one full pass over the keys and values. It also removes the unused fused reduce kernel and the shuffle segment-sort variant, and moves the row walk into a shared helper. Groups that overflow the tile or contain long rows fall back to the existing long-row path, which adds complexity and can cost extra work on skewed inputs.

Measured after the change: 37.92 billion (median of 6 runs). 13.1% lower.

```diff
diff --git a/spsparse_b200/csrc/group_sort.cuh b/spsparse_b200/csrc/group_sort.cuh
--- /dev/null
+++ b/spsparse_b200/csrc/group_sort.cuh
@@ -0,0 +1,271 @@
+#pragma once
+#include "radix_sort.cuh"
+
+constexpr int GS_THREADS = 256;
+constexpr int GS_WARPS = GS_THREADS / 32;
+constexpr int GS_CAP = 4096;
+constexpr int GS_IPT = GS_CAP / GS_THREADS;
+constexpr int GS_TILE = GS_CAP;
+constexpr int GS_MAX_BITS = 9;
+constexpr int GS_RADIX = 1 << GS_MAX_BITS;
+constexpr int GS_TC = (GS_TILE + GS_CAP) / 256 + 1;
+static_assert(GS_TILE >= GS_CAP && (1 << SG_CNT_SHIFT) == 256, "see the carry-in rule in k_group_sort");
+constexpr u32 GS_RES_DST = 0x1fffu, GS_RES_HEAD = 0x4000u, GS_RES_RHEAD = 0x8000u;
+static_assert(GS_CAP <= (int)GS_RES_DST + 1, "a destination inside the group fits GS_RES_DST");
+#ifndef GS_MIN_BLOCKS
+#define GS_MIN_BLOCKS 2
+#endif
+
+struct GsSmem {
+    u32 row[GS_CAP + 2 * SEG_MAX];
+    u32 col[GS_CAP + 2 * SEG_MAX];
+    double val[GS_CAP];
+    unsigned short res[GS_CAP];
+    u32 cnt[GS_WARPS * GS_RADIX / 2];
+    u32 hb[GS_TILE / 32];
+    u64 tc[GS_TC];
+    u32 misc[16];
+};
+
+__device__ __forceinline__ u32 gs_next_head(const u32 *hb, u32 from, u32 len) {
+    const u32 lane = threadIdx.x & 31, nw = (len + 31) >> 5;
+    for (u32 w0 = from >> 5; w0 < nw; w0 += 32) {
+        const u32 w = w0 + lane;
+        u32 bits = w < nw ? hb[w] : 0u;
+        if (w == (from >> 5)) bits &= 0xffffffffu << (from & 31);
+        const u32 any = __ballot_sync(SPB_FULL_MASK, bits != 0);
+        if (any) {
+            const u32 l = __ffs(any) - 1;
+            return ((w0 + l) << 5) + __ffs(__shfl_sync(SPB_FULL_MASK, bits, l)) - 1;
+        }
+    }
+    return len;
+}
+
+__device__ void gs_leave(const u64 *__restrict__ keys_in, const double *__restrict__ vals_in, u64 lo, u64 hi, u64 gkey,
+                         bool starts_group, int keep_all, u64 base, u64 *keys_out, double *vals_out, unsigned char *flags,
+                         u32 *long_count, u64 *tc) {
+    const u32 tid = threadIdx.x;
+    for (u64 j = lo + tid; j < hi; j += GS_THREADS) {
+        if (flags) { keys_out[j] = keys_in[j]; vals_out[j] = vals_in[j]; flags[j] = 1; }
+        else { keys_out[j] = gkey; vals_out[j] = 0.0; }
+    }
+    if (tid == 0) atomicAdd(long_count, (u32)(hi - lo));
+    const u64 t0 = lo >> SG_CNT_SHIFT, t1 = (hi - 1) >> SG_CNT_SHIFT;
+    for (u64 t = t0 + tid; t <= t1; t += GS_THREADS) {
+        u64 c = 0;
+        if (keep_all) c = min(hi, (t + 1) << SG_CNT_SHIFT) - max(lo, t << SG_CNT_SHIFT);
+        else if (starts_group && t == t0) c = 1;
+        if (starts_group && t == t0) c |= 1ull << 31;
+        if (c) atomicAdd((ull *)&tc[t - (base >> SG_CNT_SHIFT)], (ull)c);
+    }
+}
+
+__global__ void __launch_bounds__(GS_THREADS, GS_MIN_BLOCKS) k_group_sort(const u64 *__restrict__ keys_in, const double *__restrict__ vals_in,
+                                                                         const u32 *n_ptr, int bits_lo, int gbits, u64 *keys_out, double *vals_out,
+                                                                         unsigned char *flags, u32 *long_count, u64 *tile_cnt, int keep_all) {
+    extern __shared__ __align__(16) unsigned char gs_raw[];
+    GsSmem &S = *reinterpret_cast<GsSmem *>(gs_raw);
+    const u32 n = *n_ptr;
+    const u64 base = (u64)blockIdx.x * GS_TILE;
+    if (base >= n) return;
+    const u32 tid = threadIdx.x, lane = tid & 31, warp = tid >> 5;
+    const u32 tlen = n - base < (u64)GS_TILE ? (u32)(n - base) : (u32)GS_TILE;
+    const int gshift = bits_lo + gbits;
+    const u32 lo_mask = bits_lo >= 32 ? 0xffffffffu : (1u << bits_lo) - 1u;
+    const u32 gmask = (1u << gbits) - 1u;
+
+    u32 *s_grp = S.row;
+    if (tid == 0) s_grp[0] = base ? (u32)(keys_in[base - 1] >> gshift) : 0xffffffffu;
+    for (int t = tid; t < GS_TC; t += GS_THREADS) S.tc[t] = 0;
+#pragma unroll
+    for (int k = 0; k < GS_IPT; ++k) {
+        const u32 i = (u32)k * GS_THREADS + tid;
+        if (i < tlen) s_grp[1 + i] = (u32)(ld_stream_u64(keys_in + base + i) >> gshift);
+    }
+    __syncthreads();
+#pragma unroll
+    for (int k = 0; k < GS_IPT; ++k) {
+        const u32 i = (u32)k * GS_THREADS + tid;
+        const u32 hb = __ballot_sync(SPB_FULL_MASK, i < tlen && s_grp[1 + i] != s_grp[i]);
+        if (lane == 0) S.hb[i >> 5] = hb;
+    }
+    __syncthreads();
+    u32 cs = gs_next_head(S.hb, 0, tlen);
+    if (cs > 0) {
+        const u32 grp = s_grp[1];
+        bool over = cs == tlen && base + tlen < n;
+        if (!over) {
+            const u64 ge = base + cs;
+            over = ge > (u64)GS_CAP && (u32)(keys_in[ge - GS_CAP - 1] >> gshift) == grp;
+        }
+        if (over) gs_leave(keys_in, vals_in, base, base + cs, (u64)grp << gshift, false, keep_all, base, keys_out, vals_out, flags, long_count, S.tc);
+    }
+
+    while (cs < tlen) {
+        const u64 gs = base + cs;
+        const u32 grp = (u32)(keys_in[gs] >> gshift);
+        const u64 gkey = (u64)grp << gshift;
+        const u32 nx = gs_next_head(S.hb, cs + 1, tlen);
+        u64 ge = base + nx;
+        if (nx == tlen && base + tlen < n) {
+            const u64 hs = base + tlen, lim = min((u64)n, gs + GS_CAP + 1);
+            u32 first = (u32)(lim - hs);
+#pragma unroll
+            for (int k = 0; k < GS_IPT; ++k) {
+                const u64 j = hs + (u64)k * GS_THREADS + tid;
+                if (j < lim && (u32)(ld_stream_u64(keys_in + j) >> gshift) != grp) first = min(first, (u32)(j - hs));
+            }
+            first = __reduce_min_sync(SPB_FULL_MASK, first);
+            if (lane == 0) S.misc[8 + warp] = first;
+            __syncthreads();
+            first = S.misc[8];
+#pragma unroll
+            for (int w = 1; w < GS_WARPS; ++w) first = min(first, S.misc[8 + w]);
+            ge = hs + first;
+        }
+        if (ge - gs > (u64)GS_CAP) {
+            gs_leave(keys_in, vals_in, gs, base + tlen, gkey, true, keep_all, base, keys_out, vals_out, flags, long_count, S.tc);
+            break;
+        }
+        const u32 m = (u32)(ge - gs);
+        const u32 K = (m + GS_THREADS - 1) / GS_THREADS;
+        __syncthreads();
+
+        u32 dig[GS_IPT], col[GS_IPT];
+        u32 valid_bits = 0;
+#pragma unroll
+        for (int k = 0; k < GS_IPT; ++k) {
+            const u32 i = warp * 32 * K + (u32)k * 32 + lane;
+            const bool ok = (u32)k < K && i < m;
+            const u64 key = ok ? ld_stream_u64(keys_in + gs + i) : 0;
+            dig[k] = (u32)(key >> bits_lo) & gmask;
+            col[k] = (u32)key & lo_mask;
+            valid_bits |= (ok ? 1u : 0u) << k;
+            if (ok && (lane & 15) == 0) asm volatile("prefetch.global.L2 [%0];" ::"l"(vals_in + gs + i));
+        }
+        for (int t = tid; t < GS_WARPS * GS_RADIX / 2; t += GS_THREADS) S.cnt[t] = 0;
+        if (tid < (u32)SEG_MAX) { S.row[tid] = 0xffffffffu; S.row[SEG_MAX + m + tid] = 0xffffffffu; }
+        __syncthreads();
+
+        unsigned short *mycnt = reinterpret_cast<unsigned short *>(S.cnt) + warp * GS_RADIX;
+        const u32 lt = lanemask_lt();
+        unsigned short pos[GS_IPT];
+#pragma unroll
+        for (int k = 0; k < GS_IPT; ++k) {
+            pos[k] = 0;
+            if (__any_sync(SPB_FULL_MASK, (valid_bits >> k) & 1u)) {
+                const bool ok = (valid_bits >> k) & 1u;
+                u32 peers = __ballot_sync(SPB_FULL_MASK, ok);
+#pragma unroll
+                for (int b = 0; b < GS_MAX_BITS; ++b) {
+                    int sgn;
+                    asm("bfe.s32 %0, %1, %2, 1;" : "=r"(sgn) : "r"(dig[k]), "r"(b));
+                    const u32 mb = __ballot_sync(SPB_FULL_MASK, sgn != 0);
+                    peers &= ~(mb ^ (u32)sgn);
+                }
+                const u32 leader = ok ? (u32)(__ffs(peers) - 1) : lane;
+                u32 before = 0;
+                if (ok && lane == leader) {
+                    before = mycnt[dig[k]];
+                    mycnt[dig[k]] = (unsigned short)(before + __popc(peers));
+                }
+                before = __shfl_sync(SPB_FULL_MASK, before, leader);
+                pos[k] = (unsigned short)(before + __popc(peers & lt));
+                __syncwarp();
+            }
+        }
+        __syncthreads();
+
+        {
+            u32 tot0 = 0, tot1 = 0;
+#pragma unroll
+            for (int w = 0; w < GS_WARPS; ++w) {
+                const u32 c = S.cnt[w * (GS_RADIX / 2) + tid];
+                tot0 += c & 0xffffu;
+                tot1 += c >> 16;
+            }
+            const u32 pair = tot0 + tot1, incl = warp_incl_scan(pair);
+            if (lane == 31) S.misc[warp] = incl;
+            __syncthreads();
+            u32 run0 = incl - pair;
+            for (u32 w = 0; w < warp; ++w) run0 += S.misc[w];
+            u32 run1 = run0 + tot0;
+#pragma unroll
+            for (int w = 0; w < GS_WARPS; ++w) {
+                const u32 c = S.cnt[w * (GS_RADIX / 2) + tid];
+                S.cnt[w * (GS_RADIX / 2) + tid] = (run0 & 0xffffu) | (run1 << 16);
+                run0 += c & 0xffffu;
+                run1 += c >> 16;
+            }
+        }
+        __syncthreads();
+
+        {
+#pragma unroll
+            for (int k = 0; k < GS_IPT; ++k) {
+                if ((valid_bits >> k) & 1u) {
+                    const u32 p = (u32)mycnt[dig[k]] + pos[k];
+                    pos[k] = (unsigned short)p;
+                    S.row[SEG_MAX + p] = dig[k];
+                    S.col[SEG_MAX + p] = col[k];
+                }
+            }
+            double v[GS_IPT];
+#pragma unroll
+            for (int k = 0; k < GS_IPT; ++k) {
+                const u32 i = warp * 32 * K + (u32)k * 32 + lane;
+                v[k] = ((valid_bits >> k) & 1u) ? ld_stream_f64(vals_in + gs + i) : 0.0;
+            }
+#pragma unroll
+            for (int k = 0; k < GS_IPT; ++k)
+                if ((valid_bits >> k) & 1u) S.val[pos[k]] = v[k];
+        }
+        __syncthreads();
+
+        bool any_long = false;
+#pragma unroll 1
+        for (u32 p = tid; p < m; p += GS_THREADS) {
+            u32 b, f, before, same;
+            const bool is_long = sg_row_walk(S.row, S.col, SEG_MAX + p, b, f, before, same);
+            any_long |= is_long;
+            S.res[p] = (unsigned short)(((p - b + before) & GS_RES_DST) |
+                                        (keep_all || same == 0 ? GS_RES_HEAD : 0u) |
+                                        (before == 0 ? GS_RES_RHEAD : 0u));
+        }
+        const bool left = __syncthreads_or(any_long);
+        if (left) gs_leave(keys_in, vals_in, gs, ge, gkey, true, keep_all, base, keys_out, vals_out, flags, long_count, S.tc);
+#pragma unroll
+        for (int k = 0; k < GS_IPT; ++k) {
+            const u32 p0 = (u32)k * GS_THREADS + warp * 32, p = p0 + lane;
+            if (!__any_sync(SPB_FULL_MASK, !left && p < m)) continue;
+            u32 cnt_at = 0, cnt_before = 0, cnt_after = 0;
+            if (p < m) {
+                const u32 r = S.res[p];
+                const u64 d = gs + (r & GS_RES_DST);
+                keys_out[d] = gkey | ((u64)S.row[SEG_MAX + p] << bits_lo) | S.col[SEG_MAX + p];
+                vals_out[d] = S.val[p];
+                if (flags) flags[gs + p] = 0;
+                const u32 inc = ((r & GS_RES_HEAD) ? 1u : 0u) | ((r & GS_RES_RHEAD) ? 0x10000u : 0u);
+                const u64 t = d >> SG_CNT_SHIFT, tw = (gs + p0) >> SG_CNT_SHIFT;
+                if (t < tw) cnt_before = inc;
+                else if (t > tw) cnt_after = inc;
+                else cnt_at = inc;
+            }
+            const u32 a0 = __reduce_add_sync(SPB_FULL_MASK, cnt_at), a1 = __reduce_add_sync(SPB_FULL_MASK, cnt_before),
+                      a2 = __reduce_add_sync(SPB_FULL_MASK, cnt_after);
+            if (lane == 0) {
+                u64 *t = S.tc + (((gs + p0) >> SG_CNT_SHIFT) - (base >> SG_CNT_SHIFT));
+                if (a0) atomicAdd((ull *)t, (ull)(a0 & 0xffffu) | ((ull)(a0 >> 16) << 31));
+                if (a1) atomicAdd((ull *)(t - 1), (ull)(a1 & 0xffffu) | ((ull)(a1 >> 16) << 31));
+                if (a2) atomicAdd((ull *)(t + 1), (ull)(a2 & 0xffffu) | ((ull)(a2 >> 16) << 31));
+            }
+        }
+        cs = nx;
+    }
+    if (tile_cnt) {
+        __syncthreads();
+        for (int t = tid; t < GS_TC; t += GS_THREADS)
+            if (S.tc[t]) atomicAdd((ull *)(tile_cnt + (base >> SG_CNT_SHIFT) + t), (ull)S.tc[t]);
+    }
+}
diff --git a/spsparse_b200/csrc/radix_sort.cuh b/spsparse_b200/csrc/radix_sort.cuh
--- a/spsparse_b200/csrc/radix_sort.cuh
+++ b/spsparse_b200/csrc/radix_sort.cuh
@@ -544,6 +544,27 @@
 #define SGW_UNROLL_N 8
 #endif
 constexpr int SGW_UNROLL = SGW_UNROLL_N;
+
+__device__ __forceinline__ bool sg_row_walk(const u32 *s_row, const u32 *s_col, u32 q, u32 &b, u32 &f, u32 &before, u32 &same) {
+    const u32 row = s_row[q], col = s_col[q];
+    before = same = 0;
+    if (s_row[q - SEG_MAX] == row || s_row[q + SEG_MAX] == row) b = f = (u32)SEG_MAX;
+    else {
+#pragma unroll SGW_UNROLL
+        for (b = 0; b < (u32)SEG_MAX; ++b) {
+            if (s_row[q - 1 - b] != row) break;
+            const u32 c = s_col[q - 1 - b];
+            before += c <= col;
+            same += c == col;
+        }
+#pragma unroll SGW_UNROLL
+        for (f = 0; f < (u32)SEG_MAX; ++f) {
+            if (s_row[q + 1 + f] != row) break;
+            before += s_col[q + 1 + f] < col;
+        }
+    }
+    return b == (u32)SEG_MAX || f == (u32)SEG_MAX || b + f + 1 > (u32)SEG_MAX;
+}
 __global__ void __launch_bounds__(SG_THREADS, 6) k_segment_sort_walk(const u64 *__restrict__ keys_in, const double *__restrict__ vals_in,
                                                              const u32 *n_ptr, int bits_lo, u64 *keys_out, double *vals_out,
                                                              unsigned char *flags, u32 *long_count, u64 *tile_cnt = nullptr,
@@ -585,23 +606,8 @@
         bool head = true, rhead = false;
         if (g < n) {
             const u32 row = s_row[q], col = s_col[q];
-            u32 b = 0, f = 0, before = 0, same = 0;
-            if (s_row[q - SEG_MAX] == row || s_row[q + SEG_MAX] == row) b = f = (u32)SEG_MAX;
-            else {
-#pragma unroll SGW_UNROLL
-                for (b = 0; b < (u32)SEG_MAX; ++b) {
-                    if (s_row[q - 1 - b] != row) break;
-                    const u32 c = s_col[q - 1 - b];
-                    before += c <= col;
-                    same += c == col;
-                }
-#pragma unroll SGW_UNROLL
-                for (f = 0; f < (u32)SEG_MAX; ++f) {
-                    if (s_row[q + 1 + f] != row) break;
-                    before += s_col[q + 1 + f] < col;
-                }
-            }
-            const bool is_long = b == (u32)SEG_MAX || f == (u32)SEG_MAX || b + f + 1 > (u32)SEG_MAX;
+            u32 b, f, before, same;
+            const bool is_long = sg_row_walk(s_row, s_col, q, b, f, before, same);
             if (!is_long) {
                 dst = g - b + before;
                 head = keep_all || same == 0;
@@ -631,115 +637,6 @@
     if (n_long && lane == 0) atomicAdd(long_count, n_long);
 }
 
-constexpr int SGS_ROW = 5;
-constexpr int SGS_H = SGS_ROW - 1;
-constexpr int SGS_STEP = 32 - 2 * SGS_H;
-constexpr int SGS_STEPS = (256 + SGS_STEP - 1) / SGS_STEP;
-__global__ void __launch_bounds__(SG_THREADS, 6) k_segment_sort_shfl(const u64 *__restrict__ keys_in, const double *__restrict__ vals_in,
-                                                                    const u32 *n_ptr, int bits_lo, u64 *keys_out, double *vals_out,
-                                                                    unsigned char *flags, u32 *long_count, u64 *tile_cnt = nullptr,
-                                                                    int keep_all = 0) {
-    __shared__ u32 s_row[SG_TILE + 2 * SEG_MAX];
-    __shared__ u32 s_col[SG_TILE + 2 * SEG_MAX];
-    __shared__ double s_val[SG_TILE];
-    const u32 n = *n_ptr;
-    const u64 base = (u64)blockIdx.x * SG_TILE;
-    if (base >= n) return;
-    const u32 tid = threadIdx.x, lane = tid & 31, warp = tid >> 5;
-    const u32 lo_mask = bits_lo >= 32 ? 0xffffffffu : (1u << bits_lo) - 1u;
-    for (u32 q = tid; q < SG_TILE + 2 * SEG_MAX; q += SG_THREADS) {
-        const i64 g = (i64)base + (i64)q - SEG_MAX;
-        u32 row = 0xffffffffu, col = 0;
-        if (g >= 0 && g < (i64)n) {
-            const u64 key = ld_stream_u64(keys_in + g);
-            row = (u32)(key >> bits_lo);
-            col = (u32)key & lo_mask;
-        }
-        s_row[q] = row;
-        s_col[q] = col;
-    }
-#pragma unroll
-    for (int k = 0; k < SG_IPT; ++k) {
-        const u32 e = (u32)k * SG_THREADS + tid;
-        const u64 g = base + e;
-        s_val[e] = g < n ? ld_stream_f64(vals_in + g) : 0.0;
-    }
-    __syncthreads();
-    const u64 wbase = base + (u64)warp * 256;
-    u32 n_long = 0;
-    u32 cnt_at = 0, cnt_before = 0, cnt_after = 0;
-    for (int t = 0; t < SGS_STEPS; ++t) {
-        const i32 e = t * SGS_STEP + (i32)lane - SGS_H;
-        const u32 q = (u32)(SEG_MAX + (i32)warp * 256 + e);
-        const u64 g = wbase + (u64)(i64)e;
-        const bool mine = lane >= (u32)SGS_H && lane < (u32)(32 - SGS_H) && e < 256 && g < n;
-        const u32 row = s_row[q], col = s_col[q];
-        const u32 hb = __ballot_sync(SPB_FULL_MASK, s_row[q - 1] != row);
-        const u32 tail = __shfl_sync(SPB_FULL_MASK, (u32)(s_row[q + 1] != row), 31);
-        const u64 z = ~((u64)hb | ((u64)tail << 32)) & 0x1ffffffffull;
-        u64 run = z;
-#pragma unroll
-        for (int d = 1; d < SGS_ROW; ++d) run &= z >> d;
-        u32 b = 0, f = 0, before = 0, same = 0;
-        if (run == 0) {
-#pragma unroll
-            for (int d = 1; d < SGS_ROW; ++d) {
-                const u32 ru = __shfl_up_sync(SPB_FULL_MASK, row, d), cu = __shfl_up_sync(SPB_FULL_MASK, col, d);
-                const u32 rd = __shfl_down_sync(SPB_FULL_MASK, row, d), cd = __shfl_down_sync(SPB_FULL_MASK, col, d);
-                const bool up = lane >= (u32)d && ru == row, dn = lane + d < 32u && rd == row;
-                b += up;
-                before += (up && cu <= col) + (dn && cd < col);
-                same += up && cu == col;
-                f += dn;
-            }
-        } else if (mine) {
-            if (s_row[q - SEG_MAX] == row || s_row[q + SEG_MAX] == row) b = f = (u32)SEG_MAX;
-            else {
-                for (b = 0; b < (u32)SEG_MAX; ++b) {
-                    if (s_row[q - 1 - b] != row) break;
-                    const u32 c = s_col[q - 1 - b];
-                    before += c <= col;
-                    same += c == col;
-                }
-                for (f = 0; f < (u32)SEG_MAX; ++f) {
-                    if (s_row[q + 1 + f] != row) break;
-                    before += s_col[q + 1 + f] < col;
-                }
-            }
-        }
-        if (mine) {
-            const bool is_long = b == (u32)SEG_MAX || f == (u32)SEG_MAX || b + f + 1 > (u32)SEG_MAX;
-            u64 dst = g;
-            bool head = true, rhead = false;
-            if (!is_long) {
-                dst = g - b + before;
-                head = keep_all || same == 0;
-                rhead = before == 0;
-            }
-            keys_out[dst] = ((u64)row << bits_lo) | col;
-            vals_out[dst] = s_val[warp * 256 + (u32)e];
-            if (flags) flags[g] = is_long;
-            n_long += is_long;
-            const u32 inc = (head ? 1u : 0u) | (rhead ? 0x10000u : 0u);
-            if (dst < wbase) cnt_before += inc;
-            else if (dst >= wbase + 256) cnt_after += inc;
-            else cnt_at += inc;
-        }
-    }
-    if (tile_cnt) {
-        const u32 a0 = __reduce_add_sync(SPB_FULL_MASK, cnt_at), a1 = __reduce_add_sync(SPB_FULL_MASK, cnt_before),
-                  a2 = __reduce_add_sync(SPB_FULL_MASK, cnt_after);
-        if (lane == 0) {
-            u64 *t = tile_cnt + (wbase >> SG_CNT_SHIFT);
-            if (a0) atomicAdd((ull *)t, (ull)(a0 & 0xffffu) | ((ull)(a0 >> 16) << 31));
-            if (a1) atomicAdd((ull *)(t - 1), (ull)(a1 & 0xffffu) | ((ull)(a1 >> 16) << 31));
-            if (a2) atomicAdd((ull *)(t + 1), (ull)(a2 & 0xffffu) | ((ull)(a2 >> 16) << 31));
-        }
-    }
-    n_long = __reduce_add_sync(SPB_FULL_MASK, n_long);
-    if (n_long && lane == 0) atomicAdd(long_count, n_long);
-}
-
 __global__ void k_gather_flagged(const u64 *__restrict__ keys, const double *__restrict__ vals, const unsigned char *__restrict__ flags,
                                  const u64 *__restrict__ slot, u32 n, u64 *k_out, double *v_out) {
     for (u64 e = (u64)blockIdx.x * blockDim.x + threadIdx.x; e < n; e += (u64)gridDim.x * blockDim.x)
diff --git a/spsparse_b200/csrc/reduce_segsort.cuh b/spsparse_b200/csrc/reduce_segsort.cuh
--- a/spsparse_b200/csrc/reduce_segsort.cuh
+++ /dev/null
@@ -1,194 +0,0 @@
-#pragma once
-#include "radix_sort.cuh"
-#include "reduce_by_key.cuh"
-
-constexpr int RF_H = SEG_MAX;
-constexpr int RF_W = RK_TILE + 2 * RF_H;
-constexpr int RF_ITS = (RF_W + RK_THREADS - 1) / RK_THREADS;
-constexpr int RF_SORTED = RK_TILE + RF_H + 1;
-constexpr int RF_SLOTS = RF_SORTED + (RF_SORTED >> 3) + 1;
-
-struct RfSmem {
-    u64 raw[RF_W];
-    u64 keys[RF_SLOTS];
-    double vals[RF_SLOTS];
-    u64 warp[RK_WARPS];
-    u64 excl;
-    u32 tile;
-};
-
-__global__ void __launch_bounds__(RK_THREADS, 4) k_reduce_segsort(ReduceArgs a, u32 *seg_long) {
-    extern __shared__ __align__(16) unsigned char rf_smem[];
-    RfSmem &s = *reinterpret_cast<RfSmem *>(rf_smem);
-    const u32 tid = threadIdx.x, lane = tid & 31, warp = tid >> 5;
-    const bool want_rows = a.row_start != nullptr;
-    if (tid == 0) s.tile = atomicAdd(a.ticket, 1u);
-    __syncthreads();
-    const u32 tile = s.tile;
-    const u32 n = *a.n_ptr;
-    const u64 base = (u64)tile * RK_TILE;
-    if (base >= n) return;
-    const u32 tile_n = (n - base < (u64)RK_TILE) ? (u32)(n - base) : (u32)RK_TILE;
-
-    double v[RF_ITS];
-#pragma unroll
-    for (int k = 0; k < RF_ITS; ++k) {
-        const u32 q = (u32)k * RK_THREADS + tid;
-        const i64 g = (i64)base + (i64)q - RF_H;
-        const bool in = q < (u32)RF_W && g >= 0 && g < (i64)n;
-        if (q < (u32)RF_W) s.raw[q] = in ? ld_stream_u64(a.keys + g) : ~0ull;
-        v[k] = in ? ld_stream_f64(a.vals + g) : 0.0;
-    }
-    __syncthreads();
-
-    const u64 lo_mask = (1ull << a.bits_lo) - 1;
-    u32 n_long = 0;
-#pragma unroll
-    for (int k = 0; k < RF_ITS; ++k) {
-        const u32 q = (u32)k * RK_THREADS + tid;
-        if (q >= (u32)RF_W) continue;
-        const u64 key = s.raw[q];
-        if (key == ~0ull) continue;
-        const u64 row = key >> a.bits_lo, col = key & lo_mask;
-        u32 b = 0, f = 0, before = 0;
-        bool cut = false;
-        for (; b < (u32)SEG_MAX; ++b) {
-            if (q < 1 + b) { cut = true; break; }
-            const u64 kk = s.raw[q - 1 - b];
-            if ((kk >> a.bits_lo) != row) break;
-            before += (kk & lo_mask) <= col;
-        }
-        for (; f < (u32)SEG_MAX; ++f) {
-            if (q + 1 + f >= (u32)RF_W) { cut = true; break; }
-            const u64 kk = s.raw[q + 1 + f];
-            if ((kk >> a.bits_lo) != row) break;
-            before += (kk & lo_mask) < col;
-        }
-        const bool is_long = b == (u32)SEG_MAX || f == (u32)SEG_MAX || b + f + 1 > (u32)SEG_MAX;
-        if (q >= (u32)RF_H && q < (u32)(RF_H + RK_TILE)) n_long += is_long;
-        const u32 place = (cut || is_long) ? q : q - b + before;
-        if (place + 1 >= (u32)RF_H && place + 1 < (u32)(RF_H + RF_SORTED)) {
-            const u32 L = place + 1 - (u32)RF_H;
-            s.keys[rk_phys(L)] = key;
-            s.vals[rk_phys(L)] = v[k];
-        }
-    }
-    n_long = __reduce_add_sync(SPB_FULL_MASK, n_long);
-    if (n_long && lane == 0) atomicAdd(seg_long, n_long);
-    __syncthreads();
-
-    const u32 first = tid * RK_IPT;
-    const u32 mine = first < tile_n ? (tile_n - first < (u32)RK_IPT ? tile_n - first : (u32)RK_IPT) : 0;
-    u64 key[RK_IPT];
-    double acc[RK_IPT];
-    u32 head_bits = 0, rhead_bits = 0;
-    if (mine) {
-        const u64 prev = s.keys[rk_phys(first)];
-#pragma unroll
-        for (int j = 0; j < RK_IPT; ++j) {
-            key[j] = s.keys[rk_phys(first + j + 1)];
-            acc[j] = s.vals[rk_phys(first + j + 1)];
-        }
-        int cur = -1;
-#pragma unroll
-        for (int j = 0; j < RK_IPT; ++j) {
-            if ((u32)j < mine) {
-                const u64 before = j ? key[j - 1] : prev;
-                const bool head = (a.policy == POLICY_KEEP_ALL) || (base + first + j == 0) || (key[j] != before);
-                if (head) {
-                    head_bits |= 1u << j;
-                    if (want_rows && ((base + first + j == 0) || (key[j] >> a.bits_lo) != (before >> a.bits_lo)))
-                        rhead_bits |= 1u << j;
-                    cur = j;
-                } else if (cur >= 0) {
-                    const double vj = acc[j];
-#pragma unroll
-                    for (int h = 0; h < RK_IPT; ++h)
-                        if (h == cur) {
-                            if (a.policy == POLICY_ADD) acc[h] = __dadd_rn(acc[h], vj);
-                            else if (a.policy == POLICY_REPLACE) acc[h] = vj;
-                        }
-                }
-            }
-        }
-        if (cur >= 0 && mine == (u32)RK_IPT && (a.policy == POLICY_ADD || a.policy == POLICY_REPLACE)) {
-            const u64 k0 = key[RK_IPT - 1];
-            double sum = 0.0;
-#pragma unroll
-            for (int h = 0; h < RK_IPT; ++h) if (h == cur) sum = acc[h];
-            u64 q = base + first + RK_IPT;
-            while (q < n) {
-                const u32 L = (u32)(q - base) + 1;
-                if (L >= (u32)RF_SORTED) break;
-                if (s.keys[rk_phys(L)] != k0) break;
-                const double vq = s.vals[rk_phys(L)];
-                if (a.policy == POLICY_ADD) sum = __dadd_rn(sum, vq); else sum = vq;
-                ++q;
-            }
-#pragma unroll
-            for (int h = 0; h < RK_IPT; ++h) if (h == cur) acc[h] = sum;
-        }
-    }
-    const u32 emit_bits = head_bits;
-    const u64 my = (u64)__popc(emit_bits) | ((u64)__popc(rhead_bits) << 32);
-    const u64 incl = warp_incl_scan(my);
-    if (lane == 31) s.warp[warp] = incl;
-    __syncthreads();
-    u64 wbefore = 0, total = 0;
-#pragma unroll
-    for (int w = 0; w < RK_WARPS; ++w) {
-        const u64 t = s.warp[w];
-        if ((u32)w < warp) wbefore += t;
-        total += t;
-    }
-    const u64 before_me = wbefore + incl - my;
-    const u32 tile_out = (u32)(total & 0xffffffffull);
-    if (warp == 0) {
-        const u64 packed = (total & 0xffffffffull) | ((total >> 32) << 31);
-        const u64 excl0 = lookback_exclusive(a.state, tile, packed);
-        if (lane == 0) {
-            s.excl = excl0;
-            if (base + RK_TILE >= n) {
-                const u64 fin = excl0 + packed;
-                const u32 n_out = (u32)(fin & 0x7fffffffull), n_rows = (u32)(fin >> 31);
-                *a.out_count = n_out;
-                if (want_rows) { *a.row_count = n_rows; a.row_start[n_rows] = n_out; }
-            }
-        }
-    }
-    {
-        u32 slot = (u32)(before_me & 0xffffffffull);
-#pragma unroll
-        for (int j = 0; j < RK_IPT; ++j) {
-            if ((emit_bits >> j) & 1u) {
-                s.keys[slot] = key[j];
-                s.vals[slot] = acc[j];
-                ++slot;
-            }
-        }
-    }
-    __syncthreads();
-    const u64 excl_rows = s.excl >> 31;
-    const u64 excl = s.excl & 0x7fffffffull;
-    if (rhead_bits) {
-        u32 slot = (u32)(before_me & 0xffffffffull);
-        u64 rslot = excl_rows + (before_me >> 32);
-#pragma unroll
-        for (int j = 0; j < RK_IPT; ++j) {
-            if ((emit_bits >> j) & 1u) {
-                if ((rhead_bits >> j) & 1u) {
-                    a.row_start[rslot] = (u32)(excl + slot);
-                    a.row_id[rslot] = (i32)(key[j] >> a.bits_lo);
-                    ++rslot;
-                }
-                ++slot;
-            }
-        }
-    }
-    for (u32 t = tid; t < tile_out; t += RK_THREADS) {
-        const u64 k = s.keys[t];
-        a.out_hi[excl + t] = (i32)(k >> a.bits_lo);
-        if (a.out_lo) a.out_lo[excl + t] = (i32)(k & lo_mask);
-        a.out_val[excl + t] = s.vals[t];
-    }
-}
diff --git a/spsparse_b200/csrc/spb_api.cu b/spsparse_b200/csrc/spb_api.cu
--- a/spsparse_b200/csrc/spb_api.cu
+++ b/spsparse_b200/csrc/spb_api.cu
@@ -16,8 +16,8 @@
 #include "gen.cuh"
 #include "radix_sort.cuh"
 #include "radix_sort9.cuh"
+#include "group_sort.cuh"
 #include "reduce_by_key.cuh"
-#include "reduce_segsort.cuh"
 #include "reduce_warp.cuh"
 #include "scan.cuh"
 #include "spgemm.cuh"
@@ -320,7 +320,7 @@
     CK(cudaDeviceGetAttribute(&c->sm_count, cudaDevAttrMultiProcessorCount, device));
     CK(cudaFuncSetAttribute(k_radix_pass<true>, cudaFuncAttributeMaxDynamicSharedMemorySize, (int)RS_SMEM_BYTES));
     CK(cudaFuncSetAttribute(k_radix_pass<false>, cudaFuncAttributeMaxDynamicSharedMemorySize, (int)RS_SMEM_BYTES));
-    CK(cudaFuncSetAttribute(k_reduce_segsort, cudaFuncAttributeMaxDynamicSharedMemorySize, (int)sizeof(RfSmem)));
+    CK(cudaFuncSetAttribute(k_group_sort, cudaFuncAttributeMaxDynamicSharedMemorySize, (int)sizeof(GsSmem)));
     CK(cudaFuncSetAttribute(k_radix_pass9<true>, cudaFuncAttributeMaxDynamicSharedMemorySize, (int)R9_SMEM_BYTES));
     CK(cudaFuncSetAttribute(k_radix_pass9<false>, cudaFuncAttributeMaxDynamicSharedMemorySize, (int)R9_SMEM_BYTES));
     CK(cudaFuncSetAttribute(k_radix_pass<false, true>, cudaFuncAttributeMaxDynamicSharedMemorySize, (int)RS_SMEM_BYTES));
@@ -646,7 +646,6 @@
     const bool seg_short = (double)n <= 16.0 * (double)in.extent_hi && n >= (1u << 23);
     const char *walk_env = getenv("SPB_SEGMENT_WALK");
     const bool seg_walk = walk_env ? atoi(walk_env) != 0 : (double)n <= 6.0 * (double)in.extent_hi;
-    const bool seg_shfl = walk_env && atoi(walk_env) == 2;
     const bool seg = in.bits_lo > 0 && passes_full - passes_row >= 2 &&
                      (seg_env ? atoi(seg_env) != 0 : seg_short);
     const int cover_bits = seg ? job.bits_hi : key_bits;
@@ -656,8 +655,16 @@
     const bool nine_wanted = r9_env ? atoi(r9_env) != 0 : (seg && !seg_env);
     const bool nine = nine_wanted && passes9 < passes8;
     const int digit_bits = nine ? R9_BITS : RS_RADIX_BITS;
-    const int passes = nine ? passes9 : passes8;
-    const int shift0 = seg ? in.bits_lo : 0;
+    int passes = nine ? passes9 : passes8;
+    const char *group_env = getenv("SPB_GROUP_SORT");
+    int gbits = 0;
+    if (seg && passes >= 2 && !(group_env && atoi(group_env) == 0)) {
+        const int g = job.bits_hi - digit_bits * (passes - 1);
+        const double expect = (double)n * (double)(1u << g) / (double)in.extent_hi;
+        if (expect <= 0.75 * GS_CAP && (expect >= 0.25 * GS_CAP || (group_env && atoi(group_env) != 0))) gbits = g;
+    }
+    if (gbits) --passes;
+    const int shift0 = seg ? in.bits_lo + gbits : 0;
     if (n >= (1u << 31)) return spb_fail(SPB_ERR_TOO_LARGE, "%u entries: one sort holds fewer than 2^31 (the reference's own cap, algorithm.hpp:419)", n);
     Scratch ws(ctx);
     Timer tm(ctx->stream);
@@ -699,8 +706,6 @@
     int t_p0 = t0;
     CKR(run_radix_passes(ctx, ws, 0, passes, n, counters, hist, kA, vA, kB, vB, &in0, &ks, &vs, &tm, &t_p0, shift0, digit_bits));
     const int t_passes = tm.mark();
-    const char *fused_env = getenv("SPB_FUSED_REDUCE");
-    bool fused = seg && seg_walk && fused_env && atoi(fused_env) != 0;
     u32 h[6];
     int t1 = t_passes, t2 = t_passes;
     u64 *const ks_rows = ks;
@@ -712,9 +717,9 @@
         ks = ks_rows; vs = vs_rows;
         u64 *ko = (ks == kA) ? kB : kA;
         double *vo = (vs == vA) ? vB : vA;
-        const u32 stiles = (u32)div_up(n, SG_TILE);
+        const u32 stiles = (u32)div_up(n, gbits ? GS_TILE : SG_TILE);
         u64 *tile_off = nullptr;
-        if (seg && !fused) {
+        if (seg) {
             if (!long_rows_fixed) {
                 u64 *tile_cnt = nullptr;
                 if (rw_mode == 1) {
@@ -723,7 +728,7 @@
                 }
                 const int keep_all = job.policy == POLICY_KEEP_ALL;
                 ++ctx->launches;
-                if (seg_shfl) k_segment_sort_shfl<<<stiles, SG_THREADS, 0, ctx->stream>>>(ks, vs, counters, in.bits_lo, ko, vo, nullptr, counters + 5, tile_cnt, keep_all);
+                if (gbits) k_group_sort<<<stiles, GS_THREADS, sizeof(GsSmem), ctx->stream>>>(ks, vs, counters, in.bits_lo, gbits, ko, vo, nullptr, counters + 5, tile_cnt, keep_all);
                 else if (seg_walk) k_segment_sort_walk<<<stiles, SG_THREADS, 0, ctx->stream>>>(ks, vs, counters, in.bits_lo, ko, vo, nullptr, counters + 5, tile_cnt, keep_all);
                 else k_segment_sort<<<stiles, SG_THREADS, 0, ctx->stream>>>(ks, vs, counters, in.bits_lo, ko, vo, nullptr, counters + 5, tile_cnt, keep_all);
                 CK(cudaGetLastError());
@@ -738,7 +743,7 @@
                 CKR(ws.get(&slot, (u64)n_kept + 1));
                 CK(cudaMemsetAsync(counters + 5, 0, sizeof(u32), ctx->stream));
                 ++ctx->launches;
-                if (seg_shfl) k_segment_sort_shfl<<<stiles, SG_THREADS, 0, ctx->stream>>>(ks, vs, counters, in.bits_lo, ko, vo, flags, counters + 5);
+                if (gbits) k_group_sort<<<stiles, GS_THREADS, sizeof(GsSmem), ctx->stream>>>(ks, vs, counters, in.bits_lo, gbits, ko, vo, flags, counters + 5, nullptr, 0);
                 else if (seg_walk) k_segment_sort_walk<<<stiles, SG_THREADS, 0, ctx->stream>>>(ks, vs, counters, in.bits_lo, ko, vo, flags, counters + 5);
                 else k_segment_sort<<<stiles, SG_THREADS, 0, ctx->stream>>>(ks, vs, counters, in.bits_lo, ko, vo, flags, counters + 5);
                 CKR((exclusive_scan<unsigned char, u64>(ctx, ws, flags, slot, n_kept)));
@@ -757,7 +762,7 @@
         }
         t1 = tm.mark();
 
-        const bool rwarp = !fused && (tile_off != nullptr || rw_mode == 2);
+        const bool rwarp = tile_off != nullptr || rw_mode == 2;
         const u32 rtiles = rwarp ? wtiles / RW_WARPS : (u32)div_up(n, RK_TILE);
         ReduceArgs ra;
         memset(&ra, 0, sizeof ra);
@@ -770,22 +775,17 @@
         CKR(ws.get(&ra.long_list, 2ull * ra.long_cap));
         ra.long_count = counters + 3;
         ra.row_start = row_start; ra.row_id = row_id; ra.row_count = counters + 4;
-        if (fused) {
-            ++ctx->launches, k_reduce_segsort<<<rtiles, RK_THREADS, sizeof(RfSmem), ctx->stream>>>(ra, counters + 5);
-        } else {
-            if (rwarp && tile_off) ++ctx->launches, k_reduce_warp<false><<<rtiles, RW_THREADS, 0, ctx->stream>>>(ra);
-            else if (rwarp) ++ctx->launches, k_reduce_warp<true><<<rtiles, RW_THREADS, 0, ctx->stream>>>(ra);
-            else ++ctx->launches, k_reduce_by_key<MODE_CONSOLIDATE><<<rtiles, RK_THREADS, 0, ctx->stream>>>(ra);
-            if (job.policy == POLICY_ADD || job.policy == POLICY_REPLACE)
-                ++ctx->launches, k_long_runs<<<(u32)ctx->sm_count * 4, 256, 0, ctx->stream>>>(ra);
-        }
+        if (rwarp && tile_off) ++ctx->launches, k_reduce_warp<false><<<rtiles, RW_THREADS, 0, ctx->stream>>>(ra);
+        else if (rwarp) ++ctx->launches, k_reduce_warp<true><<<rtiles, RW_THREADS, 0, ctx->stream>>>(ra);
+        else ++ctx->launches, k_reduce_by_key<MODE_CONSOLIDATE><<<rtiles, RK_THREADS, 0, ctx->stream>>>(ra);
+        if (job.policy == POLICY_ADD || job.policy == POLICY_REPLACE)
+            ++ctx->launches, k_long_runs<<<(u32)ctx->sm_count * 4, 256, 0, ctx->stream>>>(ra);
         CK(cudaGetLastError());
         t2 = tm.mark();
 
         CK(cudaMemcpyAsync(h, counters, sizeof h, cudaMemcpyDeviceToHost, ctx->stream));
         CK(cudaStreamSynchronize(ctx->stream));
         if (h[5] && !h[1] && attempt == 0 && seg) {
-            fused = false;
             long_rows_fixed = true;
             CK(cudaMemsetAsync(counters + 2, 0, 3 * sizeof(u32), ctx->stream));
             continue;
```
